# nanoporetech/qcat

Hardware: AMD Instinct MI355X
Metric: reads/sec demultiplexed (higher is better)
Workload: dtype bit planes / int16 (the reference's int32 DP as differences of neighbouring cells in boolean planes: two per difference for the barcode scan, four for the adapter scan of big batches; 16-bit lanes -- u16 / exact-integer f16 -- for the rest; all proven exact per kit by range bounds at kit creation; k

## Files before the change

### include/qcat_hip.h

```cpp
#ifndef QCAT_HIP_H
#define QCAT_HIP_H

#include <stdint.h>

#ifdef __cplusplus
extern "C" {
#endif

#define QCAT_ABI_VERSION 6

enum { QCAT_CODE_A = 0, QCAT_CODE_T = 1, QCAT_CODE_G = 2, QCAT_CODE_C = 3,
       QCAT_CODE_N = 4, QCAT_CODE_X = 5, QCAT_CODE_OTHER = 6, QCAT_CODE_PAD = 7,
       QCAT_NCODES = 7 };

enum { QCAT_MAX_TEMPLATES = 16,
       QCAT_MAX_TEMPLATE_LEN = 128,
       QCAT_MAX_TARGET_LEN = 64,
       QCAT_MAX_BARCODES = 1024,
       QCAT_MAX_WINDOW = 160 };

typedef enum qcat_status {
    QCAT_OK = 0,
    QCAT_ERR_ARG = -1,
    QCAT_ERR_UNSUPPORTED = -2,
// ... 118 lines not shown
                                const int32_t* pair_offsets, const int32_t* pair_entries,
                                const int32_t* quad_offsets, const int32_t* quad_entries);

int  qcat_ctx_create(int device, qcat_ctx** out);
void qcat_ctx_destroy(qcat_ctx* ctx);

int  qcat_scan_batch(qcat_ctx* ctx, const qcat_kit* kit,
                     const uint8_t* bases, const uint64_t* offsets, uint32_t n_reads,
                     qcat_result* out, int64_t* counts);

int  qcat_detect_kit(qcat_ctx* ctx, const qcat_kit* kit,
                     const uint8_t* bases, const uint64_t* offsets, uint32_t n_reads,
                     int64_t* votes, int64_t* first_read);

int  qcat_scan_batch_auto(qcat_ctx* ctx, const qcat_kit* kit,
                          const uint8_t* bases, const uint64_t* offsets, uint32_t n_reads,
                          qcat_result* out, int64_t* counts, int32_t* chosen_kit_slot,
                          int64_t* votes, int64_t* first_read);

int  qcat_scan_batch_auto_ptrs(qcat_ctx* ctx, const qcat_kit* kit,
                               const uint8_t* const* reads, const uint64_t* lengths, uint32_t n_reads,
                               qcat_result* out, int64_t* counts, int32_t* chosen_kit_slot,
                               int64_t* votes, int64_t* first_read);

int  qcat_scan_batches_auto_ptrs(qcat_ctx* ctx, const qcat_kit* kit, const uint8_t* const* reads, const uint64_t* lengths,
                                 uint32_t n_reads, uint32_t batch_reads, qcat_result* out, int64_t* counts,
                                 int32_t* chosen_kit_slots);

int  qcat_scan_sequences(qcat_ctx* ctx, const qcat_kit* kit,
                         const uint8_t* bases, const uint64_t* offsets, uint32_t n_seqs, qcat_result* out);

enum { QCAT_STATS_NONE = 0, QCAT_STATS_PARASAIL6 = 1, QCAT_STATS_PARASAIL5 = 3, QCAT_STATS_ROUND3 = 5 };
typedef struct qcat_alignment { int32_t score, end_query, end_ref, matches, length; } qcat_alignment;
int  qcat_sg_align(qcat_ctx* ctx, const uint8_t* queries, const uint64_t* q_offsets,
                   const uint8_t* targets, const uint64_t* t_offsets, uint32_t n,
                   int32_t gap_open, int32_t gap_extend, const int8_t* matrix , int32_t with_stats,
                   qcat_alignment* out);

int  qcat_scan_debug(qcat_ctx* ctx, const qcat_kit* kit,
                     const uint8_t* bases, const uint64_t* offsets, uint32_t n_reads,
                     qcat_result* out, int64_t* counts,
                     qcat_end_trace* traces, int16_t* bc_rows, uint32_t row_stride);

int  qcat_batch_upload(qcat_ctx* ctx, const uint8_t* bases, const uint64_t* offsets,
                       uint32_t n_reads, qcat_batch** out);
typedef struct qcat_synth_params {
    uint64_t seed;
    uint32_t n_reads;
    uint32_t insert_len;
    uint32_t lead_min, lead_max;
    float    error_rate;
    float    no_adapter_fraction;
    int32_t  tpl_5p, tpl_3p;
} qcat_synth_params;
int  qcat_batch_synthesize(qcat_ctx* ctx, const qcat_kit* kit, const qcat_synth_params* p,
                           qcat_batch** out);
void qcat_batch_destroy(qcat_batch* batch);
int  qcat_batch_info(const qcat_batch* batch, uint32_t* n_reads, uint64_t* n_bases);
int  qcat_batch_download(qcat_ctx* ctx, const qcat_batch* batch, uint8_t* bases, uint64_t* offsets);
int64_t qcat_synth_read(const qcat_kit* kit, const qcat_synth_params* p, uint64_t index,
                        uint8_t* buf, uint64_t cap);

int  qcat_scan_resident(qcat_ctx* ctx, const qcat_kit* kit, const qcat_batch* batch);
int  qcat_ctx_synchronize(qcat_ctx* ctx);
int  qcat_ctx_fetch_results(qcat_ctx* ctx, qcat_result* out, uint32_t n_reads);
int  qcat_ctx_fetch_counts(qcat_ctx* ctx, int64_t* counts, int32_t n_buckets);
void* qcat_ctx_counts_devptr(qcat_ctx* ctx);
void* qcat_ctx_results_devptr(qcat_ctx* ctx);

int  qcat_kit_partition_bins(const qcat_kit* kit);
int  qcat_batch_partition(qcat_ctx* ctx, const qcat_kit* kit, const qcat_batch* batch,
                          const qcat_result* records, uint32_t flags, qcat_batch** out);
int  qcat_ctx_fetch_partition(qcat_ctx* ctx, uint64_t* bin_first, int32_t n_bins, uint32_t* source);
void* qcat_ctx_partition_bins_devptr(qcat_ctx* ctx);
void* qcat_ctx_partition_source_devptr(qcat_ctx* ctx);

void* qcat_ctx_stream(qcat_ctx* ctx);

int64_t qcat_ctx_graph_replays(const qcat_ctx* ctx);

int qcat_ctx_barcode_bitslice_tiles(qcat_ctx* ctx, uint32_t out[3]);
int64_t qcat_ctx_tiny_ends(const qcat_ctx* ctx);
int qcat_ctx_fused_front(const qcat_ctx* ctx, uint32_t out[2]);
int64_t qcat_ctx_middle_wave_reads(qcat_ctx* ctx);

int qcat_ctx_middle_bitslice_tiles(qcat_ctx* ctx, uint32_t out[4]);

int  qcat_ctx_last_timing(qcat_ctx* ctx, const char** names, float* ms, int cap);
int  qcat_ctx_set_timing(qcat_ctx* ctx, int enabled);

int  qcat_set_option(const char* name, int64_t value);
int  qcat_clear_option(const char* name);
int  qcat_get_option(const char* name, int64_t* value);
void qcat_reset_options(void);
int  qcat_option_count(void);
const char* qcat_option_name(int index);
const char* qcat_option_doc(int index);
const char* qcat_backend(void);

typedef struct qcat_fastq qcat_fastq;
int  qcat_fastq_open(const char* path, qcat_fastq** out, uint64_t* n_reads, uint64_t* n_bytes);
void qcat_fastq_close(qcat_fastq* f);
int  qcat_fastq_read_info(const qcat_fastq* f, uint64_t r, uint64_t* title_off, uint32_t* title_len,
                          uint64_t* seq_off, uint32_t* seq_len);
typedef struct qcat_demux_opts {
    int32_t batch_size;
    int32_t kit_auto;
    int32_t trim;
    int32_t min_read_length;
    int32_t tsv;
    int32_t tsv_fd;
    int32_t out_fd;
    const char* out_dir;
    const char* const* kit_name;
    const char* const* const* bc_name;
    const int32_t* const* bc_id;
    const int32_t* const* bc2_id;
    int32_t filter_barcodes;
    int32_t stream_reader;
    uint64_t segment_bytes;
    uint64_t range_begin, range_end;
    int32_t input_fd, rest_fd;
} qcat_demux_opts;
typedef struct qcat_demux_stats {
    uint64_t n_reads, n_skipped, file_bytes;
    double parse_s, scan_s, write_s;
    double total_s;
    uint64_t next_offset;
    int32_t incomplete;
    int32_t segments;
} qcat_demux_stats;
int  qcat_fastq_demux(qcat_fastq* f, qcat_ctx* ctx, const qcat_kit* kit, const qcat_demux_opts* opts,
                      qcat_result* recs, uint8_t* skipped, qcat_demux_stats* stats);

typedef struct qcat_demux_hist {
    int32_t w0, w1;
    int64_t* barcode;
    int64_t* adapter;
    int64_t n_none;
    int64_t n_adapter_none;
} qcat_demux_hist;
int  qcat_fastq_batch_offsets(const char* path, uint32_t batch_size, uint64_t segment_bytes, uint64_t** offsets,
                              uint64_t* n_batches, uint64_t* n_reads, uint64_t* next_offset);
void qcat_free(void* p);
int  qcat_fastq_demux_stream(const char* path, qcat_ctx* ctx, const qcat_kit* kit, const qcat_demux_opts* opts,
                             qcat_demux_hist* hist, qcat_demux_stats* stats);
int  qcat_fastq_stream_count(const char* path, uint64_t segment_bytes, uint32_t batch_size, int32_t stream_reader, uint64_t* n_reads,
                             uint64_t* n_bases, uint64_t* next_offset, uint32_t* n_segments);

enum { QCAT_COMM_ID_BYTES = 128, QCAT_COMM_MAX_VALUES = 64 };
enum { QCAT_REDUCE_SUM = 0, QCAT_REDUCE_MAX = 1 };
typedef struct qcat_comm qcat_comm;
int  qcat_comm_unique_id(uint8_t* id );
int  qcat_comm_create(qcat_ctx* ctx, int n_ranks, int rank, const uint8_t* id, qcat_comm** out);
void qcat_comm_destroy(qcat_comm* comm);
int  qcat_comm_info(const qcat_comm* comm, int* n_ranks, int* rank, int* device);
int  qcat_counts_allreduce(qcat_ctx* ctx, qcat_comm* comm);
int  qcat_comm_allreduce_f64(qcat_ctx* ctx, qcat_comm* comm, double* values, int n, int op);
int  qcat_comm_barrier(qcat_ctx* ctx, qcat_comm* comm);

#ifdef __cplusplus
}
#endif
#endif
```

### qcat_amd/csrc/kernels_abs.inc

```

#include "abs_core.h"
#ifndef QCAT_ABS_NO_BUILTIN
#include "abs_generated.inc"
#endif

namespace qk {

#ifndef QCAT_ABS_TILE_DEFINED
#define QCAT_ABS_TILE_DEFINED
constexpr int ABS_TILE = 2048;
#endif
#ifndef QCAT_ABS_R
#define QCAT_ABS_R 6
#endif
constexpr int ABS_R = QCAT_ABS_R;
constexpr int ABS_MAX_ROWS = 150;
#ifndef QCAT_ABS_PLANE_WAVES
#define QCAT_ABS_PLANE_WAVES 8
#endif
constexpr int ABS_PLANE_WAVES = QCAT_ABS_PLANE_WAVES;

template <int LANE>
__device__ __forceinline__ void abs_writelane(u32 value, u32& acc) {
    asm volatile("v_writelane_b32 %0, %1, %2" : "+v"(acc) : "s"(value), "n"(LANE));
// ... 97 lines not shown
constexpr uint32_t PP_GROUPS = PP_ENDS / 32;
constexpr uint32_t PP_GSTRIDE = 32 * WIN2_WORDS + 4;
static_assert(PP_ITER * PP_THREADS == PP_ENDS * PACK_PARTS && PP_THREADS % PACK_PARTS == 0 && ABS_TILE % PP_ENDS == 0 && PP_ENDS % PK_TILE == 0 &&
              PP_GROUPS * WIN2_WORDS + PP_GROUPS <= PP_THREADS && PACK_CODES == 32, "k_pack_planes: the item arithmetic below");

template <int ENDS>
__global__ void __launch_bounds__(PP_THREADS)
k_pack_planes(const uint8_t* __restrict__ bases, const uint64_t* __restrict__ offsets, uint32_t n_reads, int max_align,
              uint8_t* __restrict__ win, int32_t* __restrict__ wlen, uint8_t* __restrict__ wspec, uint32_t* __restrict__ win2, int lazy_bytes,
              uint2* __restrict__ planes, uint32_t* __restrict__ valid, uint8_t* __restrict__ need128, uint32_t* __restrict__ tile_any) {
    __shared__ __attribute__((aligned(8))) u32 s_win[PP_GROUPS * PP_GSTRIDE];
    __shared__ u32 s_bad[PP_GROUPS];
    const uint64_t n_ends = (uint64_t)n_reads * ENDS;
    const uint64_t e0 = (uint64_t)blockIdx.x * PP_ENDS;
    const uint32_t tile = (uint32_t)(e0 / ABS_TILE), lane0 = (uint32_t)(e0 % ABS_TILE) / 32u;
    if (e0 >= n_ends) {
        if (threadIdx.x < PP_GROUPS) valid[(size_t)tile * 64 + lane0 + threadIdx.x] = 0u;
        return;
    }
    if (threadIdx.x < PP_GROUPS) s_bad[threadIdx.x] = 0u;
    __syncthreads();
    {
        const uint32_t wl = threadIdx.x / PACK_PARTS, part = threadIdx.x - wl * PACK_PARTS;
#pragma unroll
        for (uint32_t it = 0; it < PP_ITER; ++it) {
            const uint32_t el = it * (PP_THREADS / PACK_PARTS) + wl;
            const uint64_t e = e0 + el;
            uint32_t p[PACK_CODES / 16] = {0u, 0u};
            if (e < n_ends && dev_pack_part<ENDS>(bases, offsets, max_align, e, part, win, wlen, wspec, win2, lazy_bytes, p))
                atomicOr(&s_bad[el >> 5], 1u << (el & 31u));
            *reinterpret_cast<uint2*>(&s_win[(el >> 5) * PP_GSTRIDE + (el & 31u) * WIN2_WORDS + part * (PACK_CODES / 16)]) = make_uint2(p[0], p[1]);
        }
    }
    __syncthreads();
    const int rows = max_align;
    if (threadIdx.x < PP_GROUPS * WIN2_WORDS) {
        const uint32_t g = threadIdx.x % PP_GROUPS, d = threadIdx.x / PP_GROUPS;
        u32 v[32];
#pragma unroll
        for (int i = 0; i < 32; ++i) v[i] = s_win[g * PP_GSTRIDE + (uint32_t)i * WIN2_WORDS + d];
        bs_transpose32(v);
        uint2* __restrict__ dst = planes + ((size_t)tile * rows + d * 16u) * 64 + lane0 + g;
#pragma unroll
        for (int q = 0; q < 16; ++q)
            if ((int)(d * 16u) + q < rows) dst[(size_t)q * 64] = make_uint2(v[2 * q + 1], v[2 * q]);
    } else if (threadIdx.x < PP_GROUPS * WIN2_WORDS + PP_GROUPS) {
        const uint32_t g = threadIdx.x - PP_GROUPS * WIN2_WORDS;
        const uint64_t eg = e0 + g * 32u;
        const u32 in = eg >= n_ends ? 0u : (n_ends - eg >= 32u ? 0xFFFFFFFFu : (1u << (uint32_t)(n_ends - eg)) - 1u);
        const u32 ok = in & ~s_bad[g];
        valid[(size_t)tile * 64 + lane0 + g] = ok;
        if (in & ~ok) need128[eg / PK_TILE] = 1;
        if (ok) tile_any[tile] = 1;
    }
}

__device__ __forceinline__ void abs_setprio(int mode, int row, int wg) {
    if (mode == 0) return;
    const int bit = ((row >> (mode - 1)) ^ wg ^ (wg >> 3)) & 1;
    if (bit) __builtin_amdgcn_s_setprio(1); else __builtin_amdgcn_s_setprio(0);
}

template <class P, int S>
constexpr bool abs_is_n(int j) {
    if constexpr (S == 0) return P::N0[j] != 0;
    else if constexpr (S == 1) return P::N1[j] != 0;
    else return P::N[j] != 0;
}
template <class P, int S, int J = 0, int NC>
__device__ __forceinline__ void abs_set2_cols(u32 (&h)[NC][4]) {
    if constexpr (J < NC) {
        if constexpr (abs_is_n<P, S>(J)) qabs::abs_set2_n(h[J]); else qabs::abs_set2(h[J]);
        abs_set2_cols<P, S, J + 1>(h);
    }
}
template <class P, int S, int J = 0, int NC>
__device__ __forceinline__ void abs_hold2_cols(u32 (&h)[NC][4], u32 hold) {
    if constexpr (J < NC) {
        if constexpr (abs_is_n<P, S>(J)) qabs::abs_hold2_n(h[J], hold); else qabs::abs_hold2(h[J], hold);
        abs_hold2_cols<P, S, J + 1>(h, hold);
    }
}

template <class P>
__device__ __forceinline__ void abs_body(const AbsArgs& A) {
    using namespace qabs;
    constexpr int NH = P::NH, NT = P::NT;
    constexpr int PL = 2 + 4 * NH;
    constexpr int LR_WORDS = 2 * ABS_NF + 1;
    static_assert(NH * LR_WORDS <= ABS_R * PL, "the last-row hand-over must fit a ring buffer");
    __shared__ u32 ring[2][ABS_R * PL * 64];
    __shared__ int s_item[2][2];
    const int lane = threadIdx.x & 63, wave = uni((int)(threadIdx.x >> 6));
    const int L = A.rows;
    const int NB = (L + ABS_R - 1) / ABS_R;

    if (wave == 0) {
        u32 h[P::NC0][4];
        int tile = -1, blk = 0;
        constexpr int ABS_PF = 3;
        uint2 pf[ABS_PF];
        const uint2* __restrict__ src = A.planes + lane;
        for (int step = 0;; ++step) {
            const int buf = step & 1;
            if (tile < 0 || blk > NB) {
                for (;;) {
                    u32 t = 0;
                    if (lane == 0) t = atomicAdd(A.cursor, 1u);
                    t = (u32)uni((int)t);
                    if (t >= A.n_tiles) { tile = -1; break; }
                    if (A.tile_any[t]) { tile = (int)t; break; }
                }
                blk = 0;
                if (tile >= 0) {
                    abs_set2_cols<P, 0>(h);
                    src = A.planes + ((size_t)tile * L) * 64 + lane;
#pragma unroll
                    for (int r = 0; r < ABS_PF; ++r) pf[r] = src[(size_t)min(r, L - 1) * 64];
                }
            }
            if (lane == 0) { s_item[buf][0] = tile; s_item[buf][1] = blk; }
            if (tile < 0) { __syncthreads(); __syncthreads(); break; }
            u32* __restrict__ rb = ring[buf];
            if (blk < NB) {
#pragma unroll 1
                for (int r = 0; r < ABS_R; ++r) {
                    const int i = blk * ABS_R + r;
                    if (i < L) {
                        abs_setprio(A.prio, i, (int)blockIdx.x);
                        const uint2 c = pf[0];
#pragma unroll
                        for (int q = 0; q + 1 < ABS_PF; ++q) pf[q] = pf[q + 1];
                        pf[ABS_PF - 1] = src[(size_t)min(i + ABS_PF, L - 1) * 64];
                        u32 nq[4], ho[NH][4];
                        abs_neq_masks(c.x, c.y, nq);
                        P::row0(nq, h, ho);
                        u32* __restrict__ row = rb + r * PL * 64 + lane;
                        row[0] = c.x; row[64] = c.y;
#pragma unroll
                        for (int k = 0; k < NH; ++k)
#pragma unroll
                            for (int p = 0; p < 4; ++p) row[(2 + 4 * k + p) * 64] = ho[k][p];
                    }
                }
            } else {
                AbsLastRow lo[NH];
                P::last0(h, lo);
#pragma unroll
                for (int k = 0; k < NH; ++k) {
                    u32* __restrict__ w = rb + k * LR_WORDS * 64 + lane;
#pragma unroll
                    for (int q = 0; q < ABS_NF; ++q) { w[q * 64] = lo[k].Fr[q]; w[(ABS_NF + q) * 64] = lo[k].sum[q]; }
                    w[2 * ABS_NF * 64] = lo[k].newmax;
                }
            }
            ++blk;
            __syncthreads();
        }
    } else {
        u32 h[P::NC1][4];
        AbsBorder bd[NT];
        __syncthreads();
        for (int step = 1;; ++step) {
            const int buf = (step - 1) & 1;
            const int tile = uni(s_item[buf][0]), blk = uni(s_item[buf][1]);
            if (tile < 0) { __syncthreads(); break; }
            const u32* __restrict__ rb = ring[buf];
            if (blk == 0) {
                abs_set2_cols<P, 1>(h);
#pragma unroll
                for (int t = 0; t < NT; ++t) {
#pragma unroll
                    for (int q = 0; q < ABS_NF; ++q) bd[t].Fc[q] = 0u;
#pragma unroll
                    for (int q = 0; q < ABS_NI; ++q) bd[t].ic[q] = 0u;
                }
            }
            if (blk < NB) {
#pragma unroll 1
                for (int r = 0; r < ABS_R; ++r) {
                    const int i = blk * ABS_R + r;
                    if (i < L) {
                        abs_setprio(A.prio, i + 1, (int)blockIdx.x);
                        const u32* __restrict__ row = rb + r * PL * 64 + lane;
                        u32 nq[4], hi[NH][4];
                        abs_neq_masks(row[0], row[64], nq);
#pragma unroll
                        for (int k = 0; k < NH; ++k)
#pragma unroll
                            for (int p = 0; p < 4; ++p) hi[k][p] = row[(2 + 4 * k + p) * 64];
                        P::row1(nq, h, hi, bd, i == 0 ? 0xFFFFFFFFu : 0u, (unsigned)i);
                    }
                }
            } else {
                AbsLastRow li[NH], lr[NT];
#pragma unroll
                for (int k = 0; k < NH; ++k) {
                    const u32* __restrict__ w = rb + k * LR_WORDS * 64 + lane;
#pragma unroll
                    for (int q = 0; q < ABS_NF; ++q) { li[k].Fr[q] = w[q * 64]; li[k].sum[q] = w[(ABS_NF + q) * 64]; }
                    li[k].newmax = w[2 * ABS_NF * 64];
                }
                P::last1(h, li, lr);
                const u32 keep = A.valid[(size_t)tile * 64 + lane];
#pragma unroll
                for (int t = 0; t < NT; ++t) {
                    u32 val[ABS_NF + 1], endq[ABS_NI];
                    abs_decide(bd[t], lr[t], (unsigned)(L - 1), val, endq, A.r1_scalar != 0);
                    const int M = t == 0 ? P::M0 : P::M1;
                    const int den = A.den[t], tpl = A.tpl[t];
                    AdapterBest* __restrict__ out = A.bests[t] + (size_t)tile * ABS_TILE + (size_t)lane * 32;
                    for (int bit = 0; bit < 32; ++bit) {
                        if (!((keep >> bit) & 1u)) continue;
                        int v = 0, e = 0;
#pragma unroll
                        for (int q = 0; q <= ABS_NF; ++q) v |= (int)((val[q] >> bit) & 1u) << q;
#pragma unroll
                        for (int q = 0; q < ABS_NI; ++q) e |= (int)((endq[q] >> bit) & 1u) << q;
                        const int score = v - 2 * M - 1;
                        if (A.dbg_tpl) {
                            const size_t eidx = (size_t)tile * ABS_TILE + (size_t)lane * 32 + (size_t)bit;
                            A.dbg_tpl[(eidx * 2 + 0) * MAX_T + tpl] = score;
                            A.dbg_tpl[(eidx * 2 + 1) * MAX_T + tpl] = e;
                        }
                        AdapterBest best; best.raw = -1; best.den = 100; best.end = -1; best.tpl = -1;
                        if (best.raw * den < score * best.den) { best.raw = score; best.den = den; best.end = e; best.tpl = tpl; }
                        out[bit] = best;
                    }
                }
            }
            __syncthreads();
        }
    }
}

template <class P>
__global__ void __launch_bounds__(128, 2)
k_adapter_bs(AbsArgs a) { abs_body<P>(a); }

template <class P, class SS, int SI>
__device__ __forceinline__ void abs_stage(const AbsArgs& A, u32* __restrict__ rings, int (*s_item)[2]) {
    using namespace qabs;
    constexpr int NS = P::NS;
    constexpr int LR_WORDS = 2 * ABS_NF + 1;
    static_assert(LR_WORDS <= ABS_R * 4, "a last-row hand-over must fit the ring rows of its difference");
    const int lane = threadIdx.x & 63;
    const int L = A.rows;
    const int NB = (L + ABS_R - 1) / ABS_R;
    constexpr int PLI = 4 * SS::HI, PLO = 4 * SS::HO;
    u32* const ring_in = SS::NHI ? rings + (size_t)SS::RING_IN * ABS_R * 64 : rings;
    u32* const ring_out = SS::NHO ? rings + (size_t)SS::RING_OUT * ABS_R * 64 : rings;
    u32 h[SS::NC][4];
    AbsBorder bd[SS::BD];
    constexpr int ABS_PF = 3;
    uint2 pf[ABS_PF];
    const uint2* __restrict__ src = A.planes + lane;
    int tile = -1, blk = 0;
    for (int step = 0;; ++step) {
        if (step < SI) { __syncthreads(); continue; }
        if (SI == 0) {
            if (tile < 0 || blk > NB) {
                for (;;) {
                    u32 t = 0;
                    if (lane == 0) t = atomicAdd(A.cursor, 1u);
                    t = (u32)uni((int)t);
                    if (t >= A.n_tiles) { tile = -1; break; }
                    if (A.tile_any[t]) { tile = (int)t; break; }
                }
                blk = 0;
            }
            if (lane == 0) { s_item[step & 7][0] = tile; s_item[step & 7][1] = blk; }
        } else {
            tile = uni(s_item[(step - SI) & 7][0]); blk = uni(s_item[(step - SI) & 7][1]);
        }
        if (tile < 0) {
            for (int q = 0; q < NS - 1 - SI; ++q) __syncthreads();
            break;
        }
        if (blk == 0) {
            abs_set2_cols<SS, 2>(h);
#pragma unroll
            for (int t = 0; t < SS::BD; ++t) {
#pragma unroll
                for (int q = 0; q < ABS_NF; ++q) bd[t].Fc[q] = 0u;
#pragma unroll
                for (int q = 0; q < ABS_NI; ++q) bd[t].ic[q] = 0u;
            }
            src = A.planes + ((size_t)tile * L) * 64 + lane;
#pragma unroll
            for (int r = 0; r < ABS_PF; ++r) pf[r] = src[(size_t)min(r, L - 1) * 64];
        }
        const u32* __restrict__ rin = ring_in + (size_t)((step - 1) & 1) * ABS_R * PLI * 64;
        u32* __restrict__ rout = ring_out + (size_t)(step & 1) * ABS_R * PLO * 64;
        if (blk < NB) {
#pragma unroll 1
            for (int r = 0; r < ABS_R; ++r) {
                const int i = blk * ABS_R + r;
                if (i < L) {
                    const uint2 c = pf[0];
#pragma unroll
                    for (int q = 0; q + 1 < ABS_PF; ++q) pf[q] = pf[q + 1];
                    pf[ABS_PF - 1] = src[(size_t)min(i + ABS_PF, L - 1) * 64];
                    u32 nq[4], hi[SS::HI][4], ho[SS::HO][4];
                    if (SS::NHI) {
#pragma unroll
                        for (int k = 0; k < SS::HI; ++k)
#pragma unroll
                            for (int p = 0; p < 4; ++p) hi[k][p] = rin[(r * PLI + 4 * k + p) * 64 + lane];
                    }
                    abs_neq_masks(c.x, c.y, nq);
                    SS::row(nq, h, hi, ho, bd, i == 0 ? 0xFFFFFFFFu : 0u, (unsigned)i);
                    if (SS::NHO) {
#pragma unroll
                        for (int k = 0; k < SS::HO; ++k)
// ... 84 lines not shown
```

### qcat_amd/csrc/kernels_generic.inc

```

namespace qk {

constexpr int GEN_THREADS = 64;
constexpr int GEN_NEG = -(1 << 28);

struct DevAlign { int score, end_q, end_r; };

struct WinSeq {
    const uint8_t* p;
    __device__ __forceinline__ int operator()(int i) const { return p[i]; }
};
struct MidSeq {
    const uint8_t* read; int64_t len; int n; int rev; int off;
    __device__ __forceinline__ int operator()(int i) const {
        const int64_t idx = (int64_t)off + i;
        uint32_t c = rev ? dev_code_of(read[len - n - 1 - idx]) : dev_code_of(read[n + idx]);
        if (rev && c < 4) c ^= 1u;
        return (int)c;
    }
};

template <class Q>
__device__ inline DevAlign dev_sg_generic(const Q q, int L,
                                          const uint8_t* __restrict__ t, int M,
// ... 21 lines not shown
    if (cmax > a.score || (cmax == a.score && (a.end_r == M - 1 || r1_scalar))) {
        a.score = cmax; a.end_r = M - 1; a.end_q = ci - 1;
    }
    return a;
}

__device__ inline uint8_t dev_code_of_ascii(uint8_t c) {
    switch (c & 0xDF) {
        case 'A': return QCAT_CODE_A;
        case 'T': return QCAT_CODE_T;
        case 'G': return QCAT_CODE_G;
        case 'C': return QCAT_CODE_C;
        case 'N': return QCAT_CODE_N;
        case 'X': return QCAT_CODE_X;
        default: return QCAT_CODE_OTHER;
    }
}

struct SgMatrix { int8_t m[49]; };

__global__ void __launch_bounds__(GEN_THREADS)
k_sg_align(const uint8_t* __restrict__ q, const uint64_t* __restrict__ qoff, const uint8_t* __restrict__ t,
           const uint64_t* __restrict__ toff, uint32_t n, int open, int ext, SgMatrix mat, int with_stats_and_rule,
           int32_t* __restrict__ scratch , qcat_alignment* __restrict__ out) {
    const int with_stats = with_stats_and_rule & 0xFF;
    const bool r1_scalar = (with_stats_and_rule & QCAT_SG_R1_SCALAR) != 0;
    const uint32_t a = blockIdx.x * blockDim.x + threadIdx.x;
    const size_t stride = (size_t)gridDim.x * blockDim.x;
    if (a >= n) return;
    const uint8_t* s1 = q + qoff[a];
    const uint8_t* s2 = t + toff[a];
    const int L = (int)(qoff[a + 1] - qoff[a]), M = (int)(toff[a + 1] - toff[a]);
    qcat_alignment r; r.score = 0; r.end_query = -1; r.end_ref = -1; r.matches = 0; r.length = 0;
    if (L <= 0 || M <= 0 || M > MAX_TLEN) { out[a] = r; return; }
    int32_t* H = scratch + a;
    int32_t* F = H + (size_t)(MAX_TLEN + 1) * stride;
    int32_t* HM = F + (size_t)(MAX_TLEN + 1) * stride;
    int32_t* HL = HM + (size_t)(MAX_TLEN + 1) * stride;
    int32_t* FM = HL + (size_t)(MAX_TLEN + 1) * stride;
    int32_t* FL = FM + (size_t)(MAX_TLEN + 1) * stride;
    for (int j = 0; j <= M; ++j) { H[j * stride] = 0; F[j * stride] = GEN_NEG; if (with_stats) { HM[j * stride] = 0; HL[j * stride] = 0; FM[j * stride] = 0; FL[j * stride] = 0; } }
    int cmax = GEN_NEG, cfirst = 0, cm = 0, cl = 0;
    for (int i = 1; i <= L; ++i) {
        const uint8_t c1 = s1[i - 1];
        const int qc = dev_code_of_ascii(c1);
        int diag = 0, dm = 0, dl = 0, hleft = 0, hlm = 0, hll = 0, e = GEN_NEG, em = 0, el = 0;
        for (int j = 1; j <= M; ++j) {
            const uint8_t c2 = s2[j - 1];
            const int tc = dev_code_of_ascii(c2);
            if (hleft - open > e - ext) { e = hleft - open; em = hlm; el = hll + 1; } else { e = e - ext; el = el + 1; }
            const int up = H[j * stride], fo = F[j * stride];
            int f, fm = 0, fl = 0;
            if (up - open > fo - ext) { f = up - open; if (with_stats) { fm = HM[j * stride]; fl = HL[j * stride] + 1; } }
            else { f = fo - ext; if (with_stats) { fm = FM[j * stride]; fl = FL[j * stride] + 1; } }
            int h = diag + mat.m[tc * 7 + qc];
            const int qm = (with_stats == QCAT_STATS_PARASAIL5 && qc == QCAT_CODE_X) ? QCAT_CODE_OTHER : qc;
            const int tm = (with_stats == QCAT_STATS_PARASAIL5 && tc == QCAT_CODE_X) ? QCAT_CODE_OTHER : tc;
            const bool same = with_stats == QCAT_STATS_ROUND3 ? (qc == tc && (c1 | 0x20) == (c2 | 0x20)) : qm == tm;
            int hm = dm + (same ? 1 : 0), hl = dl + 1;
            if (with_stats == QCAT_STATS_ROUND3) {
                if (e > h) { h = e; hm = em; hl = el; }
                if (f > h) { h = f; hm = fm; hl = fl; }
            } else {
                if (f > h) { h = f; hm = fm; hl = fl; }
                if (e > h) { h = e; hm = em; hl = el; }
            }
            diag = up;
            if (with_stats) { dm = HM[j * stride]; dl = HL[j * stride]; HM[j * stride] = hm; HL[j * stride] = hl; FM[j * stride] = fm; FL[j * stride] = fl; }
            H[j * stride] = h; F[j * stride] = f;
            hleft = h; hlm = hm; hll = hl;
        }
        if (hleft > cmax) { cmax = hleft; cfirst = i; cm = hlm; cl = hll; }
    }
    int score = GEN_NEG, end_q = L - 1, end_r = 0, mm = 0, ll = 0;
    for (int j = 1; j <= M; ++j) {
        const int v = H[j * stride];
        if (v > score) { score = v; end_r = j - 1; if (with_stats) { mm = HM[j * stride]; ll = HL[j * stride]; } }
    }
    if (cmax > score || (cmax == score && (end_r == M - 1 || r1_scalar))) { score = cmax; end_r = M - 1; end_q = cfirst - 1; mm = cm; ll = cl; }
    r.score = score; r.end_query = end_q; r.end_ref = end_r; r.matches = with_stats ? mm : 0; r.length = with_stats ? ll : 0;
    out[a] = r;
}

__device__ __host__ inline void dev_region(int tpl_len, int bc_end, int bc_len, int ext, int stop, int L,
                                           int* start_out, int* len_out) {
    int end_ref = stop - (tpl_len - bc_end) + 1;
    int start_ref = end_ref - bc_len;
    start_ref -= (ext < start_ref) ? ext : start_ref;
    end_ref += (ext < L - end_ref) ? ext : (L - end_ref);
    int a = start_ref, b = end_ref + 1;
    if (a < 0) { a += L; if (a < 0) a = 0; }
    if (b < 0) { b += L; if (b < 0) b = 0; }
    if (a > L) a = L;
    if (b > L) b = L;
    *start_out = a;
    *len_out = b > a ? b - a : 0;
}

__global__ void __launch_bounds__(GEN_THREADS)
k_scan_generic(KitPtrs kp, const uint8_t* __restrict__ win, const int32_t* __restrict__ wlen,
               uint32_t n_ends, EndRec* __restrict__ recs,
               int32_t* __restrict__ dbg_tpl ,
               int16_t* __restrict__ dbg_rows , uint32_t stride,
               int adapter_only) {
    __shared__ int H[(MAX_TLEN + 1) * GEN_THREADS];
    __shared__ int F[(MAX_TLEN + 1) * GEN_THREADS];
    __shared__ int8_t amat[49], bmat[49];
    const DevKit* k = kp.kit;
    if (threadIdx.x < 49) { amat[threadIdx.x] = k->amat[threadIdx.x]; bmat[threadIdx.x] = k->bmat[threadIdx.x]; }
    __syncthreads();
    uint32_t e = blockIdx.x * GEN_THREADS + threadIdx.x;
    if (e >= n_ends) return;
    int* h = H + threadIdx.x;
    int* f = F + threadIdx.x;
    const uint8_t* w = win + (size_t)e * WIN_STRIDE;
    const int L = wlen[e];

    int best = -1, best_end = -1, best_raw = -1, best_den = 100;
    if (L > 0) {
        for (int t = 0; t < k->nt; ++t) {
            const DevTpl& p = k->tpl[t];
            DevAlign a = dev_sg_generic(WinSeq{w}, L, kp.codes + p.code_off, p.len, k->gap_open, k->gap_extend, amat, h, f, k->r1_scalar != 0);
            if (dbg_tpl) {
                dbg_tpl[((size_t)e * 2 + 0) * MAX_T + t] = a.score;
                dbg_tpl[((size_t)e * 2 + 1) * MAX_T + t] = a.end_q;
            }
            if ((int64_t)best_raw * p.den < (int64_t)a.score * best_den) {
                best = t; best_end = a.end_q; best_raw = a.score; best_den = p.den;
            }
        }
    }
    EndRec r;
    r.window_len = L; r.best_tpl = best; r.best_end = best_end; r.best_raw = best_raw;
    r.used_tpl = best < 0 ? k->nt - 1 : best;
    const DevTpl& p = k->tpl[r.used_tpl];
    const bool dual = k->mode == QCAT_MODE_DUAL;
    r.region_path = (dual || p.is_double || (best >= 0 && best_raw >= p.region_min_raw)) ? 1 : 0;
    for (int s = 0; s < 2; ++s) { r.region_start[s] = 0; r.region_len[s] = 0; r.bc_idx[s] = -1; r.bc_raw[s] = 0; }
    const int nsets = adapter_only ? 0 : (dual ? 2 : 1);
    for (int s = 0; s < nsets; ++s) {
        if (r.region_path) dev_region(p.len, p.bc_end[s], p.bc_len[s], k->ext, best_end, L, &r.region_start[s], &r.region_len[s]);
        else { r.region_start[s] = 0; r.region_len[s] = L < k->max_align ? L : k->max_align; }
        const DevSet& bs = p.sets[s];
        int bi = -1, braw = 0;
        if (r.region_len[s] > 0) {
            for (int b = 0; b < bs.n; ++b) {
                DevAlign a = dev_sg_generic(WinSeq{w + r.region_start[s]}, r.region_len[s],
                                            kp.codes + bs.tgt_off + (size_t)b * bs.tlen, bs.tlen, 1, 1, bmat, h, f);
                if (dbg_rows) dbg_rows[((size_t)e * 2 + s) * stride + b] = (int16_t)a.score;
                if (bi < 0 || braw == 0 || braw < a.score) { bi = b; braw = a.score; }
            }
        }
        r.bc_idx[s] = bi; r.bc_raw[s] = braw;
    }
    recs[e] = r;
}

template <class MakeQ>
__device__ inline EndRec dev_scan_any(const KitPtrs& kp, MakeQ make_q, int m, int kit_slot,
                                      const int8_t* amat, const int8_t* bmat, int* h, int* f) {
    const DevKit* k = kp.kit;
    const int n = k->max_align;
    int best = -1, best_end = -1, best_raw = -1, best_den = 100, last = -1;
    for (int t = 0; t < k->nt; ++t) {
        const DevTpl& p = k->tpl[t];
        if (kit_slot >= 0 && p.kit_slot != kit_slot) continue;
        last = t;
        if (m <= 0) continue;
        DevAlign a = dev_sg_generic(make_q(0), m, kp.codes + p.code_off, p.len,
                                    k->gap_open, k->gap_extend, amat, h, f, k->r1_scalar != 0);
        if ((int64_t)best_raw * p.den < (int64_t)a.score * best_den) { best = t; best_end = a.end_q; best_raw = a.score; best_den = p.den; }
    }
    EndRec r;
    r.window_len = m; r.best_tpl = best; r.best_end = best_end; r.best_raw = best_raw;
    r.used_tpl = best < 0 ? last : best;
    const DevTpl& p = k->tpl[r.used_tpl];
    const bool dual = k->mode == QCAT_MODE_DUAL;
    r.region_path = (dual || p.is_double || (best >= 0 && best_raw >= p.region_min_raw)) ? 1 : 0;
    const int nsets = dual ? 2 : 1;
    for (int s = 0; s < 2; ++s) { r.region_start[s] = 0; r.region_len[s] = 0; r.bc_idx[s] = -1; r.bc_raw[s] = 0; }
// ... 133 lines not shown
```

### qcat_amd/csrc/kernels_packed.inc

```

#include "cols_generated.inc"

namespace qk {

typedef unsigned short us2 __attribute__((ext_vector_type(2)));
typedef short ss2 __attribute__((ext_vector_type(2)));
typedef uint32_t u32;

__device__ __forceinline__ us2 as_us2(u32 x) { return __builtin_bit_cast(us2, x); }
__device__ __forceinline__ u32 as_u32(us2 x) { return __builtin_bit_cast(u32, x); }
__device__ __forceinline__ us2 pkmax(us2 a, us2 b) { return __builtin_elementwise_max(a, b); }
__device__ __forceinline__ us2 pkmin(us2 a, us2 b) { return __builtin_elementwise_min(a, b); }
__device__ __forceinline__ us2 pkmax_i16(us2 a, us2 b) {
    return __builtin_bit_cast(us2, __builtin_elementwise_max(__builtin_bit_cast(ss2, a), __builtin_bit_cast(ss2, b)));
}
__device__ __forceinline__ us2 pksubsat(us2 a, us2 b) { return __builtin_elementwise_sub_sat(a, b); }
__device__ __forceinline__ us2 addp(us2 a, us2 b) { return as_us2(as_u32(a) + as_u32(b)); }
__device__ __forceinline__ us2 splat(u32 v) { return as_us2(v | (v << 16)); }
__device__ __forceinline__ us2 pack2(u32 lo, u32 hi) { return as_us2(lo | (hi << 16)); }
__device__ __forceinline__ int uni(int v) { return __builtin_amdgcn_readfirstlane(v); }
__device__ __forceinline__ u32 to_vgpr(u32 s) { u32 v; asm volatile("v_mov_b32 %0, %1" : "=v"(v) : "s"(s)); return v; }
__device__ __forceinline__ u32 opaque_v(u32 x) { asm volatile("" : "+v"(x)); return x; }

__device__ __forceinline__ int wave_max(int v) {
#pragma unroll
    for (int off = 32; off > 0; off >>= 1) v = max(v, __shfl_xor(v, off, 64));
    return uni(v);
}

typedef _Float16 h2 __attribute__((ext_vector_type(2)));
__device__ __forceinline__ h2 as_h2(u32 x) { return __builtin_bit_cast(h2, x); }
__device__ __forceinline__ u32 as_u32(h2 x) { return __builtin_bit_cast(u32, x); }
__device__ __forceinline__ h2 hsplat(float v) { const _Float16 x = (_Float16)v; return h2{x, x}; }
__device__ __forceinline__ h2 hmax(h2 a, h2 b) { return __builtin_elementwise_maximum(a, b); }
__device__ __forceinline__ h2 hmin(h2 a, h2 b) { return __builtin_elementwise_minimum(a, b); }
__device__ __forceinline__ h2 hmax3(h2 a, h2 b, h2 c) { return __builtin_elementwise_maximum(__builtin_elementwise_maximum(a, b), c); }
__device__ __forceinline__ u32 make_sel_h(u32 qb) {
    return ((((qb << 12) | qb) & 0x000F000Fu) << 8) | 0x000C000Cu;
}

constexpr int PK_WAVES = 1;
constexpr int PK_TILE = 128;
constexpr int PK_ROWS = 152;
constexpr int JOB_CLASSES = 7;
constexpr int JOB_HOT = 3;
constexpr int JOB_GROUPS = MAX_T * 2;
constexpr int JOB_BINS = JOB_GROUPS * JOB_CLASSES;
static_assert(JOB_BINS <= 256, "a bin index is one byte of a job word (k_adapter_finish)");

__device__ __host__ __forceinline__ int job_class(int L) { return L <= 48 ? 0 : (L <= 64 ? 1 : (L <= 96 ? 2 : 3)); }
__device__ __forceinline__ int job_class_hot_of(int bs_ok, int max_align, int bs_off, int hot_len, int short_min, int flag, int L, int start) {
    if ((flag == 0 || flag == 2) && bs_ok && bs_off >= 0) {
        const bool interior = flag == 2;
        if (L == max_align && (!interior || start == 0)) return JOB_CLASSES - 1;
        if (L == hot_len && !interior) return JOB_CLASSES - 2;
        if (L < hot_len && L >= short_min && !interior) return JOB_CLASSES - 3;
    }
    return job_class(L);
}
__device__ __forceinline__ u32 make_sel(u32 qb) {
    return (((qb << 12) | qb) & 0x000F000Fu) | 0x0C000C00u;
}

#define QK_SEL_KEY_LO 0x0C050400u
#define QK_SEL_KEY_HI 0x0C070600u

struct JobTables {
    uint32_t hist[JOB_BINS];
    uint32_t cursor[JOB_BINS];
    uint32_t group_tile_start[JOB_GROUPS + 1];
    uint32_t unit_cursor[JOB_GROUPS][8][32];
};

enum { TBL_VGPR = 1, TBL_LDS = 2 };

#define QK_POOL(J) (((J) <= PADMAX) ? spv[((J) <= PADMAX) ? (J) - 1 : 0] : special)

template <int W, int TBL>
__device__ __forceinline__ void adapter_align(const u32* __restrict__ tsrc, int M, int g, int Lmax,
                                              const uint8_t* qbuf, int lane, us2 gL2, u32 special,
                                              u32 sel_klo, u32 sel_khi, u32* ltbl, u32 (&rk)[2], u32 (&ck)[2]) {
    const int start = W - M;
    u32 tbl[TBL == TBL_LDS ? 1 : W];
    if constexpr (TBL == TBL_LDS) {
        for (int j = lane; j < W; j += 64) ltbl[j] = tsrc[j];
    } else {
#pragma unroll
        for (int j = 0; j < W; ++j) tbl[j] = tsrc[j];
#pragma unroll
        for (int j = 0; j < W; ++j) tbl[j] = opaque_v(tbl[j]);
    }
    u32 spv[PADMAX];
#pragma unroll
    for (int j = 0; j < PADMAX; ++j) spv[j] = (j + 1 > start) ? special : 0u;
    us2 h[W + 1];
    const us2 g2 = as_us2(opaque_v(as_u32(splat((u32)g))));
    {
        us2 r = splat((u32)(-(g * start)) & 0xFFFFu);
        h[0] = splat(0);
#pragma unroll
        for (int j = 1; j <= W; ++j) { r = r + g2; h[j] = pkmax_i16(r, splat(0)); }
    }
    ck[0] = ck[1] = 0;
    us2 h0old = splat(0);
    u32 qb = qbuf[lane];
    for (int i = 1; i <= Lmax; ++i) {
        if constexpr (TBL == TBL_LDS) asm volatile("" ::: "memory");
        const u32 qb_next = qbuf[(i < PK_ROWS ? i : PK_ROWS - 1) * 64 + lane];
        const u32 sel = make_sel(qb);
        const us2 h0new = pkmin(splat((u32)(g * i)), gL2);
        us2 left = h0new, carry = h0old;
#define QK_W(J) as_us2(__builtin_amdgcn_perm(QK_POOL(J), (TBL == TBL_LDS ? ltbl[(J) - 1] : tbl[TBL == TBL_LDS ? 0 : (J) - 1]), sel))
#define QK_FENCE() if constexpr (TBL == TBL_LDS) asm volatile("" ::: "memory");
#define QK_T us2
#define QK_ADD(a, b) addp(a, b)
#define QK_MAX3(d, u, l) pkmax(pkmax(d, u), l)
        QK_ROW_COLS_DISPATCH(W)
#undef QK_MAX3
#undef QK_ADD
#undef QK_T
#undef QK_FENCE
#undef QK_W
        const u32 dcol = as_u32(left - h0new);
        const u32 ci = (u32)(255 - i);
        ck[0] = max(ck[0], __builtin_amdgcn_perm(dcol, ci, sel_klo));
        ck[1] = max(ck[1], __builtin_amdgcn_perm(dcol, ci, sel_khi));
        h0old = h0new;
        qb = qb_next;
    }
    rk[0] = rk[1] = 0;
    {
        us2 r = splat((u32)(-(g * start) - 1) & 0xFFFFu);
        u32 cj = to_vgpr(255u);
#pragma unroll
        for (int j = 1; j <= W; ++j) {
            r = r + g2;
            cj -= 1u;
            const u32 v = as_u32(pksubsat(h[j], r));
            rk[0] = max(rk[0], __builtin_amdgcn_perm(v, cj, sel_klo));
            rk[1] = max(rk[1], __builtin_amdgcn_perm(v, cj, sel_khi));
        }
    }
}

struct AdapterBest { int32_t raw, den, end, tpl; };

template <int W, int TBL>
__global__ void __launch_bounds__(PK_WAVES * 64, W <= 48 ? 4 : (W <= 64 ? 3 : 2))
k_adapter_packed(KitPtrs kp, const uint8_t* __restrict__ win, const int32_t* __restrict__ wlen,
                 uint32_t n_ends, AdapterBest* __restrict__ bests,
                 int32_t* __restrict__ dbg_tpl, int use_static) {
    __shared__ uint8_t qbuf_all[PK_WAVES][PK_ROWS * 64];
    __shared__ __attribute__((aligned(16))) u32 ltbl_all[PK_WAVES][TBL == TBL_LDS ? W : 4];
    const DevKit* __restrict__ k = kp.kit;
    const int wave = threadIdx.x >> 6, lane = threadIdx.x & 63;
    uint8_t* qbuf = qbuf_all[wave];
    u32* ltbl = ltbl_all[wave];
    const uint32_t base = (blockIdx.x * PK_WAVES + wave) * PK_TILE;
    if (base >= n_ends) return;
    const uint32_t e2[2] = {base + lane, base + 64 + lane};
    const bool valid[2] = {e2[0] < n_ends, e2[1] < n_ends};
    int L2[2] = {valid[0] ? wlen[e2[0]] : 0, valid[1] ? wlen[e2[1]] : 0};

    const uint4 padv = make_uint4(0x07070707u, 0x07070707u, 0x07070707u, 0x07070707u);
    for (int c = 0; c < WIN_STRIDE / 16; ++c) {
        uint4 a = valid[0] ? *reinterpret_cast<const uint4*>(win + (size_t)e2[0] * WIN_STRIDE + c * 16) : padv;
        uint4 b = valid[1] ? *reinterpret_cast<const uint4*>(win + (size_t)e2[1] * WIN_STRIDE + c * 16) : padv;
        const u32 aw[4] = {a.x, a.y, a.z, a.w}, bw[4] = {b.x, b.y, b.z, b.w};
#pragma unroll
        for (int q = 0; q < 16; ++q) {
            const u32 lo = (aw[q >> 2] >> (8 * (q & 3))) & 0xFu;
            const u32 hi = (bw[q >> 2] >> (8 * (q & 3))) & 0xFu;
            if (c * 16 + q < PK_ROWS) qbuf[(c * 16 + q) * 64 + lane] = (uint8_t)(lo | (hi << 4));
        }
    }
    const int Lmax = wave_max(max(L2[0], L2[1]));
    const int g = uni(k->gap_open);
    const int nt = uni(k->nt);
    const us2 gL2 = pack2((u32)(g * L2[0]), (u32)(g * L2[1]));
    const u32 special = to_vgpr(k->special_adapter);
    const u32 sel_klo = to_vgpr(QK_SEL_KEY_LO), sel_khi = to_vgpr(QK_SEL_KEY_HI);

    AdapterBest best[2];
#pragma unroll
    for (int hf = 0; hf < 2; ++hf) {
        best[hf].raw = -1; best[hf].den = 100; best[hf].end = -1; best[hf].tpl = -1;
    }
    for (int t = 0; t < nt; ++t) {
        if (uni(k->tpl[t].width) != W) continue;
        if (use_static && uni(k->tpl[t].static_kernel) >= 0) continue;
        const int M = uni(k->tpl[t].len);
        const int den = uni(k->tpl[t].den);
        const u32* __restrict__ tsrc = kp.tables + uni(k->tpl[t].tbl_off);
        u32 rk[2], ck[2];
        adapter_align<W, TBL>(tsrc, M, g, Lmax, qbuf, lane, gL2, special, sel_klo, sel_khi, ltbl, rk, ck);
        const bool r1_scalar = uni(k->r1_scalar) != 0;
        const int start = W - M;
#pragma unroll
        for (int hf = 0; hf < 2; ++hf) {
            const int L = L2[hf];
            if (L > 0) {
                const int vr = (int)(rk[hf] >> 8) - 1, jr = 255 - (int)(rk[hf] & 255u) - start;
                const int vc = (int)(ck[hf] >> 8), ic = 255 - (int)(ck[hf] & 255u);
                const int s_row = vr - g * L, s_col = vc - g * M;
                const bool col = s_col > s_row || (s_col == s_row && (jr == M || r1_scalar));
                const int score = col ? s_col : s_row;
                const int endq = col ? ic - 1 : L - 1;
                if (dbg_tpl) {
                    dbg_tpl[((size_t)e2[hf] * 2 + 0) * MAX_T + t] = score;
                    dbg_tpl[((size_t)e2[hf] * 2 + 1) * MAX_T + t] = endq;
                }
                const int lhs = best[hf].raw * den, rhs = score * best[hf].den;
                if (lhs < rhs || (lhs == rhs && best[hf].tpl >= 0 && t < best[hf].tpl)) {
                    best[hf].raw = score; best[hf].den = den; best[hf].end = endq; best[hf].tpl = t;
                }
            }
        }
    }
#pragma unroll
    for (int hf = 0; hf < 2; ++hf) if (valid[hf]) bests[e2[hf]] = best[hf];
}

__global__ void __launch_bounds__(256)
k_adapter_finish(const DevKit* __restrict__ k, const int32_t* __restrict__ wlen, uint32_t n_ends,
                 const AdapterBest* __restrict__ bests, int n_slices, EndRec* __restrict__ recs,
                 JobTables* __restrict__ jt, const int32_t* __restrict__ fallback_tpl, int kit_mask,
                 const uint8_t* __restrict__ wspec, uint32_t* __restrict__ jobinfo, int2* __restrict__ bcres,
                 uint32_t* __restrict__ fin, const int32_t* __restrict__ kit_slot_dev = nullptr, uint32_t slot_span = 0) {
    if (kit_slot_dev && !slot_span) kit_mask = *kit_slot_dev;
    __shared__ uint32_t hist[JOB_BINS];
    struct FinTpl { int32_t kit_slot, is_double, region_min_raw, len, bc_end[2], bc_len[2], hot_len[2], short_min[2], bs_off[2]; };
    __shared__ FinTpl s_tpl[MAX_T];
    if (threadIdx.x < JOB_BINS) hist[threadIdx.x] = 0;
    const int nt = k->nt;
    if ((int)threadIdx.x < nt) {
        const DevTpl& p = k->tpl[threadIdx.x];
        FinTpl f;
        f.kit_slot = p.kit_slot; f.is_double = p.is_double; f.region_min_raw = p.region_min_raw; f.len = p.len;
#pragma unroll
        for (int s = 0; s < 2; ++s) {
            f.bc_end[s] = p.bc_end[s]; f.bc_len[s] = p.bc_len[s];
            f.hot_len[s] = p.sets[s].hot_len; f.short_min[s] = p.sets[s].bs_short_min; f.bs_off[s] = p.sets[s].bs_off;
        }
        s_tpl[threadIdx.x] = f;
    }
    __syncthreads();
    const bool dual = k->mode == QCAT_MODE_DUAL;
    const int nsets = dual ? 2 : 1;
    const int bs_ok = k->bs_ok, max_align = k->max_align, ext = k->ext;
    for (uint32_t e = blockIdx.x * blockDim.x + threadIdx.x; e < n_ends; e += gridDim.x * blockDim.x) {
        AdapterBest cs[MAX_T];
#pragma unroll
        for (int sl = 0; sl < MAX_T; ++sl) if (sl < n_slices) cs[sl] = bests[(size_t)sl * n_ends + e];
        const int L = wlen[e];
        const int flag = wspec ? (int)wspec[e] : 1;
        const int fb = fallback_tpl ? fallback_tpl[e] : 0;
        if (slot_span) kit_mask = kit_slot_dev[e / slot_span];
        AdapterBest b = cs[0];
        if (kit_mask >= 0 && b.tpl >= 0 && s_tpl[b.tpl].kit_slot != kit_mask) { b.raw = -1; b.den = 100; b.end = -1; b.tpl = -1; }
#pragma unroll
        for (int sl = 1; sl < MAX_T; ++sl) {
            if (sl >= n_slices) break;
            const AdapterBest c = cs[sl];
            if (c.tpl < 0) continue;
            if (kit_mask >= 0 && s_tpl[c.tpl].kit_slot != kit_mask) continue;
            const int lhs = b.raw * c.den, rhs = c.raw * b.den;
            if (lhs < rhs || (lhs == rhs && b.tpl >= 0 && c.tpl < b.tpl)) b = c;
        }
        EndRec r;
        r.window_len = L; r.best_tpl = b.tpl; r.best_end = b.end; r.best_raw = b.raw;
        int last = nt - 1;
        if (kit_mask >= 0) while (last > 0 && s_tpl[last].kit_slot != kit_mask) --last;
        r.used_tpl = b.tpl < 0 ? (fallback_tpl ? fb : last) : b.tpl;
        const FinTpl& p = s_tpl[r.used_tpl];
        r.region_path = (dual || p.is_double || (b.tpl >= 0 && b.raw >= p.region_min_raw)) ? 1 : 0;
        for (int s = 0; s < 2; ++s) { r.region_start[s] = 0; r.region_len[s] = 0; r.bc_idx[s] = -1; r.bc_raw[s] = 0; }
        for (int s = 0; s < nsets; ++s) {
            if (r.region_path) dev_region(p.len, p.bc_end[s], p.bc_len[s], ext, b.end, L, &r.region_start[s], &r.region_len[s]);
            else { r.region_start[s] = 0; r.region_len[s] = L < max_align ? L : max_align; }
            uint32_t ji = 0;
            if (r.region_len[s] > 0 && !(fallback_tpl != nullptr && r.region_len[s] > max_align)) {
                const int bin = (r.used_tpl * 2 + s) * JOB_CLASSES +
                                job_class_hot_of(bs_ok, max_align, p.bs_off[s], p.hot_len[s], p.short_min[s], flag, r.region_len[s], r.region_start[s]);
                atomicAdd(&hist[bin], 1u);
                ji = (uint32_t)min(r.region_len[s], 255) | ((uint32_t)bin << 8) | ((uint32_t)r.region_start[s] << 16);
            }
            jobinfo[(size_t)e * nsets + s] = ji;
            if (bcres) bcres[(size_t)e * nsets + s] = make_int2(-1, 0);
        }
        if (fin) fin[e] = (uint32_t)(r.window_len & 0xFF) | ((uint32_t)(r.used_tpl & 0xFF) << 8) | ((uint32_t)(uint16_t)(int16_t)r.best_end << 16);
        else recs[e] = r;
    }
    __syncthreads();
    if (threadIdx.x < JOB_BINS && hist[threadIdx.x]) atomicAdd(&jt->hist[threadIdx.x], hist[threadIdx.x]);
}

__global__ void k_job_offsets(JobTables* jt) {
    __shared__ uint32_t s_hist[JOB_BINS], s_cur[JOB_BINS], s_grp[JOB_GROUPS + 1];
    if (blockIdx.x != 0) return;
    for (int b = (int)threadIdx.x; b < JOB_BINS; b += (int)blockDim.x) s_hist[b] = jt->hist[b];
    __syncthreads();
    if (threadIdx.x == 0) {
        uint32_t pos = 0;
        for (int gidx = 0; gidx < JOB_GROUPS; ++gidx) {
            const uint32_t gstart = pos;
            s_grp[gidx] = gstart / PK_TILE;
            for (int c = 0; c < JOB_CLASSES; ++c) {
                s_cur[gidx * JOB_CLASSES + c] = pos;
                pos += s_hist[gidx * JOB_CLASSES + c];
            }
            pos = gstart + (pos - gstart + PK_TILE - 1) / PK_TILE * PK_TILE;
        }
        s_grp[JOB_GROUPS] = pos / PK_TILE;
    }
    __syncthreads();
    for (int b = (int)threadIdx.x; b < JOB_BINS; b += (int)blockDim.x) jt->cursor[b] = s_cur[b];
    for (int g = (int)threadIdx.x; g <= JOB_GROUPS; g += (int)blockDim.x) jt->group_tile_start[g] = s_grp[g];
}

constexpr int SCAT_PER_THREAD = 8;
__global__ void __launch_bounds__(256)
k_job_scatter(const uint32_t* __restrict__ jobinfo, uint32_t n_ends, int nsets,
              JobTables* __restrict__ jt, int32_t* __restrict__ sorted, uint32_t* __restrict__ posof) {
    __shared__ uint32_t cnt[JOB_BINS], basep[JOB_BINS];
    if (threadIdx.x < JOB_BINS) cnt[threadIdx.x] = 0;
    __syncthreads();
    const uint32_t n_cand = n_ends * (uint32_t)nsets;
    const uint32_t blk0 = blockIdx.x * 256u * SCAT_PER_THREAD;
    int key[SCAT_PER_THREAD]; uint32_t rank[SCAT_PER_THREAD];
#pragma unroll
    for (int it = 0; it < SCAT_PER_THREAD; ++it) {
        const uint32_t id = blk0 + it * 256u + threadIdx.x;
        key[it] = -1; rank[it] = 0;
        if (id < n_cand) {
            const uint32_t ji = jobinfo[id];
            if (ji) {
                key[it] = (int)((ji >> 8) & 0xFFu);
                rank[it] = atomicAdd(&cnt[key[it]], 1u);
            }
        }
    }
    __syncthreads();
    if (threadIdx.x < JOB_BINS && cnt[threadIdx.x]) basep[threadIdx.x] = atomicAdd(&jt->cursor[threadIdx.x], cnt[threadIdx.x]);
    __syncthreads();
#pragma unroll
    for (int it = 0; it < SCAT_PER_THREAD; ++it)
    {
        const uint32_t id = blk0 + it * 256u + threadIdx.x;
        if (key[it] >= 0) {
            const uint32_t pos = basep[key[it]] + rank[it];
            sorted[pos] = (int32_t)id;
            if (posof) posof[id] = pos;
        } else if (posof && id < n_cand) posof[id] = 0xFFFFFFFFu;
    }
}

struct TileMeta { uint32_t e_lo, e_hi, len2, pad; };
struct BsPlan;
__device__ __forceinline__ bool bs_covers(const BsPlan* __restrict__ bp, int gidx, uint32_t tile);
__device__ __forceinline__ void bs_uncovered_runs(const BsPlan* __restrict__ bp, uint32_t t0, uint32_t t1, int gidx, uint32_t (&start)[4], uint32_t (&len)[4]);

constexpr int GATHER_THREADS = 64 * (WIN_STRIDE / 16);
__global__ void __launch_bounds__(GATHER_THREADS)
k_job_gather(const uint8_t* __restrict__ win, const uint32_t* __restrict__ jobinfo, const int32_t* __restrict__ sorted,
             const JobTables* __restrict__ jt, int nsets, uint8_t* __restrict__ tilebuf, TileMeta* __restrict__ tmeta,
             const BsPlan* __restrict__ taken ,
             const uint32_t* __restrict__ win2 = nullptr, const uint8_t* __restrict__ wspec = nullptr ) {
    const uint32_t chunks = WIN_STRIDE / 16;
    const uint32_t chunk = threadIdx.x % chunks, lane = threadIdx.x / chunks;
    const uint32_t n_tiles = jt->group_tile_start[JOB_GROUPS];
    auto image = [&](uint32_t tile) {
        const int32_t id2[2] = {sorted[(size_t)tile * PK_TILE + lane], sorted[(size_t)tile * PK_TILE + 64 + lane]};
        uint32_t e2[2] = {0, 0};
        int L2[2] = {0, 0}, st2[2] = {0, 0};
#pragma unroll
        for (int hf = 0; hf < 2; ++hf) {
            if (id2[hf] >= 0) {
// ... 385 lines not shown
        __syncthreads();
        if (threadIdx.x == 0) {
            int bi = -1, braw = 0;
            for (int b = 0; b < bs.n; ++b) {
                const int raw = score[b];
                if (bi < 0 || braw == 0 || braw < raw) { bi = b; braw = raw; }
            }
            if (bcres) bcres[(size_t)e * (k->mode == QCAT_MODE_DUAL ? 2 : 1) + set] = make_int2(bi, braw);
            else { recs[e].bc_idx[set] = bi; recs[e].bc_raw[set] = braw; }
        }
        __syncthreads();
    }
}

constexpr int QCAT_JIT_BASE = 1 << 20;
enum { QCAT_JIT_ADAPTER = 0, QCAT_JIT_MIDDLE = 1, QCAT_JIT_BARCODE = 2, QCAT_JIT_BITSLICE = 3,
       QCAT_JIT_ABS2 = 4, QCAT_JIT_ABSM = 5, QCAT_JIT_ABSW = 6 };
#ifndef QCAT_RTC
static inline void jit_launch(int kind, int index, dim3 grid, hipStream_t stream, const void* args);
#endif

struct StaticArgs {
    KitPtrs kp;
    const uint8_t* tilebuf;
    const TileMeta* tmeta;
    JobTables* jt;
    u32* raws;
    int bstride, chunk_b, gidx, xcd_queues;
    u32* part;
    int part_stride;
    const BsPlan* bs;
};
struct StaticBarcodeMulti {
    StaticArgs common;
    int16_t gidx[JOB_GROUPS], chunk_b[JOB_GROUPS];
    int16_t kernel[JOB_GROUPS];
    int32_t n;
};
#ifndef QCAT_RTC
static inline void launch_barcode_static(int kernel, dim3 grid, hipStream_t stream, const StaticArgs& a);
static inline void launch_barcode_multi(dim3 grid, hipStream_t stream, const StaticBarcodeMulti& m);
#endif
struct StaticAdapterArgs {
    KitPtrs kp;
    const uint8_t* win;
    const int32_t* wlen;
    uint32_t n_ends;
    AdapterBest* bests;
    int32_t* dbg_tpl;
    int tpl;
    AdapterBest* bests2;
    int tpl2;
    const uint8_t* only;
    const uint32_t* win2;
    const uint8_t* wspec;
};

struct FillList { int32_t n; uint32_t word[8]; void* p[8]; unsigned long long bytes[8]; };
__global__ void __launch_bounds__(256)
k_fill_multi(FillList f) {
    for (int r = 0; r < f.n; ++r) {
        const unsigned long long n16 = f.bytes[r] / 16;
        const uint4 v = make_uint4(f.word[r], f.word[r], f.word[r], f.word[r]);
        uint4* __restrict__ q = reinterpret_cast<uint4*>(f.p[r]);
        for (unsigned long long i = (unsigned long long)blockIdx.x * blockDim.x + threadIdx.x; i < n16; i += (unsigned long long)gridDim.x * blockDim.x) q[i] = v;
        const unsigned tail = (unsigned)(f.bytes[r] - n16 * 16);
        if (blockIdx.x == 0 && threadIdx.x < tail) reinterpret_cast<uint8_t*>(f.p[r])[n16 * 16 + threadIdx.x] = (uint8_t)f.word[r];
    }
}

struct AbsArgs {
    const uint2* planes;
    const uint32_t* valid;
    const uint32_t* tile_any;
    AdapterBest* bests[2];
    int32_t tpl[2];
    int32_t den[2];
    uint32_t n_ends, n_tiles;
    int32_t rows;
    uint32_t* cursor;
    int32_t* dbg_tpl;
    int32_t prio;
    int32_t r1_scalar;
};
struct StaticAdapterMulti {
    StaticAdapterArgs common;
    AdapterBest* bests[MAX_T];
    AdapterBest* bests2[MAX_T];
    int16_t tpl[MAX_T], tpl2[MAX_T];
    int16_t kernel[MAX_T];
    int16_t fused[MAX_T];
};
#ifndef QCAT_RTC
static inline void launch_adapter_static(int kernel, dim3 grid, hipStream_t stream, const StaticAdapterArgs& a);
static inline void launch_adapter_fused(int kernel, dim3 grid, hipStream_t stream, const StaticAdapterArgs& a);
static inline void launch_adapter_multi(dim3 grid, hipStream_t stream, const StaticAdapterMulti& m);
#endif

}
```

### qcat_amd/csrc/options.h

```cpp
#ifndef QCAT_OPTIONS_H
#define QCAT_OPTIONS_H
#ifndef QCAT_RTC
#include <atomic>
#include <stdint.h>
#include <stdlib.h>

#define QCAT_OPTION_LIST(X) \
    X(NO_STATIC, "1: no generated static-letter kernels (binary16 table kernels instead)") \
    X(NO_STATIC_ADAPTER, "1: the adapter templates on the table kernels") \
    X(NO_FUSED_ADAPTER, "1: the two templates of a kit as two launches instead of the fused kernel") \
    X(NO_BARCODE_MULTI, "1: the static-letter barcode kernels of a small batch as launches of their own instead of one (k_barcode_multi)") \
    X(NO_ADAPTER_MULTI, "1: the static-letter adapter kernels of a small batch as launches of their own instead of one (k_adapter_multi)") \
    X(BARCODE_U16, "1 at kit creation: u16 lanes instead of exact-integer binary16 for the barcode tables") \
    X(NO_BITSLICE, "1: every barcode alignment on the binary16 kernels") \
    X(NO_BS_STATIC, "1: bit-sliced barcode kernels with the letters from memory") \
    X(BITSLICE_MIN, "barcode alignments from which the bit-sliced path is taken (default: 40 000 + 1 900 000 / barcodes; dual kits 70 000 + 3 500 000 / barcodes)") \
    X(BITSLICE_PAD, "jobs from which the rest of a hot class becomes a padded super-tile (0 / unset: never)") \
    X(BS_NO_SOLO, "1: no producer waves for the shared columns") \
    X(BS_NO_SHORT, "1: regions a few bases short of nominal stay on the binary16 kernels (no front-padded units)") \
    X(BS_SIDE, "1: ... on side streams whatever the batch size") \
    X(LEFTOVER_SIDE, "0 / 1: the left-over binary16 tiles behind / beside the bit-sliced launches") \
    X(BS_DRAW, "0 / 1: the waves of a bit-sliced workgroup take a unit's barcodes round robin / draw them from a counter (default 1; sets of 32 barcodes or more)") \
    X(BS_TRACE, "1: print the phase boundaries of one workgroup and the unit log of the bit-sliced launches") \
    X(BS_TRACE_UNITS, "1: ... and every unit") \
    X(BS_TRACE_WG, "the workgroup whose phase boundaries BS_TRACE prints (default 0)") \
    X(BS_TRACE_SEQ, "... from its n-th unit on (eight units; default 0)") \
    X(CHUNK_BARCODES, "barcodes per work unit of the binary16 barcode kernels") \
    X(ONE_QUEUE, "1: one unit queue instead of XCD-local ones") \
    X(ONE_STREAM, "1: no side streams") \
    X(RAWS, "1: keep the per-barcode raw score array (no summary keys)") \
    X(SUMMARY, "1: summary keys for small barcode sets as well") \
    X(NO_ADAPTER_BITSLICE, "1: the adapter scan on the binary16 kernels") \
    X(ADAPTER_BITSLICE_MIN, "read ends from which the bit-sliced adapter scan is taken") \
    X(ABS_STAGES, "2 / 4: one form of the adapter plans for every batch size") \
    X(FORCE_GENERIC, "1 at context creation: the general int32 kernel for everything") \
    X(MIDDLE_GENERIC, "1: --detect-middle on the general kernel") \
    X(MIDDLE_NO_ABS, "1: the interior adapter scan on the binary16 kernel") \
    X(MIDDLE_ABS_MIN, "slots from which the bit-sliced interior adapter scan is taken") \
    X(MIDDLE_ABS_ROWS, "rows of the interior's plane buffer") \
    X(MIDDLE_ABS_ONE_WAVE, "0 / 1: two-wave pipeline / one wave per big tile") \
    X(NO_PIPELINE, "1: no chunked host pipeline") \
    X(PIPELINE_CHUNK, "reads per chunk of the host pipeline") \
    X(PIPELINE_TRACE, "1: print the split of a pipelined call") \
    X(NO_SIMPLE_PACKED, "1: simple mode on the general kernel (k_scan_simple) instead of the packed end-tracking kernels") \
    X(NO_TINY, "1: batches of a handful of read ends take the throughput kernels like every other batch") \
    X(TINY_MAX_ENDS, "largest batch (read ends, at most 4096) on the one-wave-per-alignment kernels (default: by the number of alignments, 20000)") \
    X(WAVE_MAX, "most alignments of a call (pairs of qcat_sg_align without statistics; sequences of qcat_scan_sequences with affine gap costs, sequences x barcodes with a simple list) that take the one-wave kernels (default: the limits in kernels_tiny.inc)") \
    X(AUTO_CHUNK, "batches per call of the kit-auto file loop") \
    X(AUTO_WORKERS, "contexts of the kit-auto file loop") \
    X(NO_GRAPH, "1: host-buffer calls never replay a captured graph") \
    X(DEBUG_VOTE, "1: print the kit vote") \
    X(DEBUG_BINS, "1: print the jobs per length class") \
    X(DEBUG_REDO, "1: print how many alignments took the sequential arg-max")

#define QCAT_AB_OPTION_LIST(X) \
    X(NO_QUADS, "1 at kit creation: static barcode chains as pairs only") \
    X(BS_STATIC_MIN, "super-tiles from which the generated bit-sliced kernels are taken") \
    X(BS_FROM_TILES, "1: bit-sliced units read tile images instead of the two-bit windows") \
    X(BS_NO_TAIL_SPLIT, "1: the last round of long units is not cut into barcode chunks") \
    X(BS_SERIAL, "1: the bit-sliced launches of a scan in line on the context's stream") \
    X(NO_SLIM, "1: the 60-byte per-end records instead of the packed result arrays") \
    X(NO_FILL_MERGE, "1: one fill launch per buffer instead of k_fill_multi") \
    X(EAGER_BYTES, "1: byte windows for every read end, not only for those with a letter outside A, C, G, T") \
    X(PACK_PLANES, "0: windows and adapter letter planes of a big batch as two kernels (k_pack_windows, k_abs_planes) instead of one (k_pack_planes)") \
    X(FIN_BLOCKS, "blocks of k_finalize") \
    X(FINISH_BLOCKS, "blocks of k_adapter_finish") \
    X(ABS_NO_SPLIT, "1: medium batches keep the fused two-template plan") \
    X(ABS_PRIO, "issue priority rotation of the bit-sliced adapter kernels") \
    X(ADAPTER_REVERSE, "1: the side-by-side adapter launches in reverse order") \
    X(MIDDLE_NO_BITSLICE, "1: the interior's barcode jobs on the binary16 kernels") \
    X(MIDDLE_ABS_WINDOWS, "0: the M-ends' first windows from the reads instead of the packed batch") \
    X(MIDDLE_ABS_WGS, "workgroups per CU of the interior adapter kernels") \
    X(MIDDLE_ABS_EARLY, "1: the packed batch at the start of the scan") \
    X(MIDDLE_ABS_PRIO, "issue priority rotation of the interior adapter kernels") \
    X(FULL_UPLOAD, "1: host-buffer calls upload whole reads") \
    X(ABS_SERIAL, "1: the bit-sliced adapter launches of a scan one after the other instead of side by side (A/B)") \
    X(NO_ZERO_COPY, "1: host-buffer calls of a handful of reads copy their staging to the device like bigger ones (A/B)") \
    X(STREAM_SYNC_RELEASE, "1: the file loop's reader gives a written segment's pages back itself (A/B: a thread of its own)")

enum QcatOpt {
#define X(N, D) QO_##N,
    QCAT_OPTION_LIST(X)
    QO_PUBLIC_COUNT,
    QO_AB_BASE_ = QO_PUBLIC_COUNT - 1,
    QCAT_AB_OPTION_LIST(X)
#undef X
    QO_COUNT
};
#ifdef QCAT_AB
constexpr int QO_SETTABLE = QO_COUNT;
#else
constexpr int QO_SETTABLE = QO_PUBLIC_COUNT;
#endif

constexpr int64_t QOPT_UNSET = INT64_MIN;
extern std::atomic<int64_t> g_qcat_opt[QO_COUNT];

struct QOptVal {
    bool set;
    int64_t v;
    explicit operator bool() const { return set; }
};
inline QOptVal qopt_get(QcatOpt o) { if ((int)o >= QO_SETTABLE) return QOptVal{false, 0}; const int64_t v = g_qcat_opt[o].load(std::memory_order_relaxed); return QOptVal{v != QOPT_UNSET, v == QOPT_UNSET ? 0 : v}; }
inline bool opt_is_set(QcatOpt o) { return (int)o < QO_SETTABLE && g_qcat_opt[o].load(std::memory_order_relaxed) != QOPT_UNSET; }
inline bool opt_on(QcatOpt o) { if ((int)o >= QO_SETTABLE) return false; const int64_t v = g_qcat_opt[o].load(std::memory_order_relaxed); return v != QOPT_UNSET && v != 0; }
inline int64_t opt_val(QcatOpt o, int64_t dflt) { if ((int)o >= QO_SETTABLE) return dflt; const int64_t v = g_qcat_opt[o].load(std::memory_order_relaxed); return v == QOPT_UNSET ? dflt : v; }
inline int atoi(const QOptVal& o) { return (int)o.v; }
inline long long atoll(const QOptVal& o) { return (long long)o.v; }
#endif
#endif
```

### qcat_amd/csrc/packed_host.inc

```

#include "dev_buf.h"

extern "C" void qcat_abs_launch_planes(unsigned n_tiles, void* stream, const uint32_t* win2, const int32_t* wlen, const uint8_t* wspec,
                                       uint32_t n_ends, int rows, void* planes, uint32_t* valid, uint8_t* need128, uint32_t* tile_any);
extern "C" unsigned qcat_abs_launch_pack_planes(void* stream, const uint8_t* bases, const uint64_t* offsets, uint32_t n_reads, int ends, int rows,
                                                uint8_t* win, int32_t* wlen, uint8_t* wspec, uint32_t* win2, int lazy_bytes,
                                                void* planes, uint32_t* valid, uint8_t* need128, uint32_t* tile_any);
extern "C" int qcat_abs_launch(int kind, int id, unsigned grid, void* stream, const void* args);

namespace qk {

#ifndef QCAT_ABS_TILE_DEFINED
#define QCAT_ABS_TILE_DEFINED
constexpr int ABS_TILE = 2048;
#endif
constexpr int RESUME_KIT_ON_DEVICE = 1 << 20;

struct PackedScratch {
    DevBuf<JobTables> jt;
    DevBuf<int32_t> sorted;
    DevBuf<uint32_t> jobinfo;
    DevBuf<AdapterBest> bests;
    int n_slices = 0;
    bool slices_single = false;
    DevBuf<uint8_t> tilebuf;
    DevBuf<TileMeta> tmeta;
    DevBuf<uint32_t> raws;
    DevBuf<uint32_t> part;
    DevBuf<uint32_t> redo;
    const uint8_t* wspec = nullptr;
    const uint8_t* win = nullptr;
    const uint32_t* win2 = nullptr;
    bool lazy = false;
    DevBuf<BsPlan> bsplan;
    DevBuf<uint32_t> bskeys;
    bool bs_last = false;
    DevBuf<uint2> bsrp;
    DevBuf<uint2> abs_planes;
    DevBuf<uint32_t> abs_valid;
    DevBuf<uint8_t> abs_flags;
    DevBuf<uint32_t> posof;
    DevBuf<int2> bcres;
    bool slim = false;
    DevBuf<uint32_t> fin;
    bool fin_only = false;
    uint32_t abs_ready = 0;
    uint32_t abs_zeroed = 0;
    const int32_t* kit_slot_dev = nullptr;
    uint32_t kit_slot_span = 0;
    bool prepared = false;
    bool redo_zeroed = false;
    static constexpr int NAUX = 11;
    hipStream_t aux[NAUX] = {};
    hipEvent_t ev_fork = nullptr, ev_join[NAUX] = {};
};

static thread_local std::string g_packed_err;
static thread_local FillList g_fill = {};
static thread_local bool g_fill_defer = false;
static inline hipError_t packed_fill(void* p, int byte, size_t bytes, hipStream_t stream) {
    if (g_fill_defer && g_fill.n < 8 && bytes > 0) {
        const uint32_t b = (uint32_t)(byte & 0xFF);
        g_fill.p[g_fill.n] = p; g_fill.bytes[g_fill.n] = bytes; g_fill.word[g_fill.n] = b * 0x01010101u; ++g_fill.n;
        return hipSuccess;
    }
    return bytes ? hipMemsetAsync(p, byte, bytes, stream) : hipSuccess;
}
static inline hipError_t packed_fill_flush(hipStream_t stream) {
    g_fill_defer = false;
    if (g_fill.n == 0) return hipSuccess;
    unsigned long long most = 0;
    for (int r = 0; r < g_fill.n; ++r) most = std::max(most, g_fill.bytes[r]);
    const unsigned blocks = (unsigned)std::min<unsigned long long>(1024, std::max<unsigned long long>(1, most / (16 * 256 * 4)));
    hipLaunchKernelGGL(k_fill_multi, dim3(blocks), dim3(256), 0, stream, g_fill);
    g_fill.n = 0;
    return hipGetLastError();
}
struct FillScope {
    explicit FillScope(bool defer) { g_fill.n = 0; g_fill_defer = defer; }
    ~FillScope() { g_fill.n = 0; g_fill_defer = false; }
    FillScope(const FillScope&) = delete;
    FillScope& operator=(const FillScope&) = delete;
};
static inline const char* packed_last_error() { return g_packed_err.c_str(); }
static thread_local int g_jit_rc = 0;
static inline int jit_take_error() { const int rc = g_jit_rc; g_jit_rc = 0; return rc; }

static inline hipError_t packed_streams(PackedScratch* s) {
    if (s->ev_fork) return hipSuccess;
    hipError_t e = hipEventCreateWithFlags(&s->ev_fork, hipEventDisableTiming);
    for (int i = 0; i < PackedScratch::NAUX && e == hipSuccess; ++i) {
        e = hipStreamCreateWithFlags(&s->aux[i], hipStreamNonBlocking);
        if (e == hipSuccess) e = hipEventCreateWithFlags(&s->ev_join[i], hipEventDisableTiming);
    }
    return e;
}

template <class Launch>
static inline void fork_join(PackedScratch* s, hipStream_t stream, int n, Launch launch) {
    if (n <= 0) return;
    const bool multi = n > 1 && s->ev_fork && !opt_on(QO_ONE_STREAM);
    if (multi) (void)hipEventRecord(s->ev_fork, stream);
    bool used[PackedScratch::NAUX] = {};
    for (int i = 0; i < n; ++i) {
        hipStream_t q = stream;
        if (multi && i > 0) {
            const int a = (i - 1) % PackedScratch::NAUX;
            q = s->aux[a];
            if (!used[a]) { (void)hipStreamWaitEvent(q, s->ev_fork, 0); used[a] = true; }
        }
        launch(i, q);
    }
    for (int a = 0; a < PackedScratch::NAUX; ++a)
        if (used[a]) { (void)hipEventRecord(s->ev_join[a], s->aux[a]); (void)hipStreamWaitEvent(stream, s->ev_join[a], 0); }
}

static inline void packed_streams_reset(PackedScratch* s) {
    for (int i = 0; i < PackedScratch::NAUX; ++i) {
        if (s->aux[i]) (void)hipStreamDestroy(s->aux[i]);
        if (s->ev_join[i]) (void)hipEventDestroy(s->ev_join[i]);
        s->aux[i] = nullptr; s->ev_join[i] = nullptr;
    }
    if (s->ev_fork) (void)hipEventDestroy(s->ev_fork);
    s->ev_fork = nullptr;
}

static inline void packed_scratch_free(PackedScratch* s) { packed_streams_reset(s); }

static inline int packed_max_width(const DevKit& k) {
    int m = 0;
    for (int t = 0; t < k.nt; ++t) m = std::max(m, k.tpl[t].width);
    return m;
// ... 13 lines not shown
    return (int)QCAT_ERR_DEVICE;
}
template <class T>
static inline int packed_ensure(DevBuf<T>& b, size_t n, const char* what) {
    const hipError_t e = b.ensure(n);
    return e == hipSuccess ? 0 : packed_fail(("hipMalloc(" + std::string(what) + ")").c_str(), e);
}

static inline int abs_cu_count() {
    int cus = 256, dev = 0;
    (void)hipGetDevice(&dev);
    (void)hipDeviceGetAttribute(&cus, hipDeviceAttributeMultiprocessorCount, dev);
    return cus;
}
static inline int abs_forms(const DevKit& hk, int t) {
    const int sk = hk.tpl[t].static_kernel;
    if (sk < 0) return 0;
    if (sk >= QCAT_JIT_BASE) return hk.tpl[t].abs_jit;
    return (qcat_abs_launch(1, sk, 0, nullptr, nullptr) ? 1 : 0) | (qcat_abs_launch(2, sk, 0, nullptr, nullptr) ? 2 : 0) |
           (qcat_abs_launch(3, sk, 0, nullptr, nullptr) ? 4 : 0);
}
static inline void abs_launch_form(const DevKit& hk, int t, int form, unsigned grid, hipStream_t q, const AbsArgs& aa) {
    const int sk = hk.tpl[t].static_kernel;
    if (sk >= QCAT_JIT_BASE) jit_launch(form == 1 ? QCAT_JIT_ABS2 : (form == 2 ? QCAT_JIT_ABSM : QCAT_JIT_ABSW), t, dim3(grid), q, &aa);
    else (void)qcat_abs_launch(form == 1 ? 1 : (form == 2 ? 2 : 3), sk, grid, q, &aa);
}
static inline bool packed_abs_wanted(const DevKit& hk, uint32_t n_ends, bool have_wspec) {
    const bool use_static_a = hk.adapter_f16 && !opt_on(QO_NO_STATIC) && !opt_on(QO_NO_STATIC_ADAPTER);
    const QOptVal amin = qopt_get(QO_ADAPTER_BITSLICE_MIN);
    const size_t abs_min = amin ? (size_t)atoll(amin) : (size_t)abs_cu_count() * 7 * ABS_TILE / 2;
    if (!(hk.abs_ok && have_wspec && use_static_a && !opt_on(QO_NO_ADAPTER_BITSLICE))) return false;
    const size_t abs_min_ms = (size_t)abs_cu_count() * 3 * ABS_TILE / 2;
    const bool medium = n_ends < std::max<size_t>(abs_min, 1);
    if (medium && (amin || n_ends < abs_min_ms)) return false;
    bool any = false;
    for (int t = 0; t < hk.nt; ++t) {
        const int forms = abs_forms(hk, t);
        if (medium) { if (!(forms & 2)) return false; any = true; continue; }
        if (forms & 5) any = true;
        if (hk.tpl[t].static_kernel >= 0 && hk.tpl[t].static_kernel < QCAT_JIT_BASE && hk.tpl[t].fused_kernel >= 0 &&
            qcat_abs_launch(0, hk.tpl[t].fused_kernel, 0, nullptr, nullptr) != 0) any = true;
    }
    return any;
}
static inline int packed_abs_buffers(hipStream_t stream, const DevKit& hk, uint32_t n_ends, PackedScratch* sc) {
    hipError_t e;
    int rc;
    const uint32_t abs_tiles = (n_ends + ABS_TILE - 1) / ABS_TILE;
    const size_t need_planes = (size_t)abs_tiles * hk.max_align * 64, need_valid = (size_t)abs_tiles * 64;
    const size_t need_flags = (size_t)MAX_T * 4 + (size_t)abs_tiles * 4 + (size_t)abs_tiles * (ABS_TILE / PK_TILE);
    if ((rc = packed_ensure(sc->abs_planes, need_planes, "adapter letter planes"))) return rc;
    if ((rc = packed_ensure(sc->abs_valid, need_valid, "adapter keep masks"))) return rc;
    if ((rc = packed_ensure(sc->abs_flags, need_flags, "adapter tile flags"))) return rc;
    if ((e = packed_fill(sc->abs_flags, 0, need_flags, stream)) != hipSuccess) return packed_fail("memset(adapter tile flags)", e);
    sc->abs_zeroed = n_ends;
    return 0;
}

static inline int packed_prepare(hipStream_t stream, const DevKit& hk, uint32_t n_ends, PackedScratch* sc) {
    auto fail = packed_fail;
    const int nsets = hk.mode == QCAT_MODE_DUAL ? 2 : 1;
    const size_t n_cand = (size_t)n_ends * nsets;
    const size_t need_sorted = n_cand + (size_t)JOB_GROUPS * PK_TILE;
    hipError_t e;
    int rc;
    if ((rc = packed_ensure(sc->jt, 1, "job tables"))) return rc;
    if ((e = packed_streams(sc)) != hipSuccess) return fail("side streams", e);
    if ((rc = packed_ensure(sc->sorted, need_sorted, "sorted jobs"))) return rc;
    if ((rc = packed_ensure(sc->jobinfo, n_cand, "job words"))) return rc;
    if (sc->slim) {
        if ((rc = packed_ensure(sc->posof, n_cand, "job positions"))) return rc;
        if ((rc = packed_ensure(sc->bcres, n_cand, "barcode results"))) return rc;
        if ((rc = packed_ensure(sc->fin, n_ends, "finalize words"))) return rc;
    }
    if ((e = packed_fill(sc->jt, 0, sizeof(JobTables), stream)) != hipSuccess) return fail("memset(job tables)", e);
    if ((e = packed_fill(sc->sorted, 0xFF, need_sorted * 4, stream)) != hipSuccess) return fail("memset(sorted)", e);
    if (sc->redo && (e = packed_fill(sc->redo, 0, 4, stream)) != hipSuccess) return fail("memset(redo count)", e);
    sc->redo_zeroed = sc->redo != nullptr;

    return 0;
}

static inline int packed_adapter_finish(hipStream_t stream, KitPtrs kp, const uint8_t* , const int32_t* wlen,
                                        uint32_t n_ends, EndRec* recs, PackedScratch* sc, int kit_mask) {
    const QOptVal fb_env = qopt_get(QO_FINISH_BLOCKS);
    const uint32_t fblocks = std::min<uint32_t>((n_ends + 255) / 256, fb_env ? (uint32_t)std::max(1, atoi(fb_env)) : 1024u);
    const int32_t* slot_dev = kit_mask == RESUME_KIT_ON_DEVICE ? sc->kit_slot_dev : nullptr;
    hipLaunchKernelGGL(k_adapter_finish, dim3(fblocks), dim3(256), 0, stream, kp.kit, wlen, n_ends, sc->bests, sc->n_slices, recs, sc->jt,
                       (const int32_t*)nullptr, slot_dev ? -1 : kit_mask, sc->wspec, sc->jobinfo, sc->slim ? sc->bcres : nullptr, sc->fin_only ? sc->fin : nullptr,
                       slot_dev, slot_dev ? sc->kit_slot_span : 0u);
    hipError_t e = hipGetLastError();
    if (e != hipSuccess) return packed_fail("packed kernel launch", e);
    return 0;
}

template <class Mark>
static inline int packed_adapter(hipStream_t stream, KitPtrs kp, const DevKit& hk, const uint8_t* win,
                                 const int32_t* wlen, uint32_t n_ends, EndRec* recs, PackedScratch* sc,
                                 int32_t* dbg_tpl, Mark mark) {
    auto fail = packed_fail;
    hipError_t e;
    int rc;
    const int adapter_widths[] = {40, 48, 56, 60, 64, 84, 92, 104, 112, 120, 128};
    const bool use_static_a = hk.adapter_f16 && !opt_on(QO_NO_STATIC) && !opt_on(QO_NO_STATIC_ADAPTER);
    auto table_tpl = [&](int t, int w) { return hk.tpl[t].width == w && !(use_static_a && hk.tpl[t].static_kernel >= 0); };
    int n_slices = 0, n_static_a = 0;
    for (int w : adapter_widths) { bool present = false; for (int t = 0; t < hk.nt; ++t) present |= table_tpl(t, w); n_slices += present; }
    for (int t = 0; t < hk.nt; ++t) if (use_static_a && hk.tpl[t].static_kernel >= 0) { ++n_slices; ++n_static_a; }
    if ((rc = packed_ensure(sc->bests, (size_t)n_ends * n_slices, "adapter bests"))) return rc;
    const uint32_t tiles = (n_ends + PK_TILE - 1) / PK_TILE;
    const uint32_t blocks = (tiles + PK_WAVES - 1) / PK_WAVES;
    {
        int slice = 0;
#define QK_LAUNCH(WW, TT) do { bool present = false; for (int t = 0; t < hk.nt; ++t) present |= table_tpl(t, WW); \
        if (present) { hipLaunchKernelGGL((k_adapter_packed<WW, TT>), dim3(blocks), dim3(PK_WAVES * 64), 0, stream, kp, win, wlen, n_ends, \
                                          sc->bests + (size_t)slice * n_ends, dbg_tpl, use_static_a ? 1 : 0); ++slice; } } while (0)
        QK_LAUNCH(40, TBL_VGPR); QK_LAUNCH(48, TBL_VGPR); QK_LAUNCH(56, TBL_VGPR); QK_LAUNCH(60, TBL_VGPR); QK_LAUNCH(64, TBL_VGPR);
        QK_LAUNCH(84, TBL_LDS); QK_LAUNCH(92, TBL_LDS); QK_LAUNCH(104, TBL_LDS); QK_LAUNCH(112, TBL_LDS); QK_LAUNCH(120, TBL_LDS); QK_LAUNCH(128, TBL_LDS);
#undef QK_LAUNCH
        if (slice) mark("k_adapter_packed");
        const bool use_fused = !opt_on(QO_NO_FUSED_ADAPTER);
        const uint32_t abs_tiles = (n_ends + ABS_TILE - 1) / ABS_TILE;
        const int abs_cus = abs_cu_count();
        const bool abs_wanted = packed_abs_wanted(hk, n_ends, sc->wspec != nullptr && (sc->win2 != nullptr || sc->abs_ready == n_ends));
        const bool abs_split = abs_wanted && abs_tiles < (uint32_t)abs_cus * 4u && !opt_on(QO_ABS_NO_SPLIT);
        int stpl[MAX_T], sslice[MAX_T], spartner[MAX_T], pslice[MAX_T];
        int ns = 0, nsl = 0;
        bool taken[MAX_T] = {};
        for (int t = 0; t < hk.nt; ++t) {
            if (!(use_static_a && hk.tpl[t].static_kernel >= 0) || taken[t]) continue;
            stpl[ns] = t; sslice[ns] = slice + nsl++; spartner[ns] = -1; pslice[ns] = 0;
            const int p = hk.tpl[t].fused_partner;
            const bool split_pair = abs_split && p > t && hk.tpl[t].static_kernel < QCAT_JIT_BASE &&
                                    (abs_forms(hk, t) & 1) && (abs_forms(hk, p) & 1);
            if (!split_pair && use_fused && hk.tpl[t].fused_kernel >= 0 && hk.tpl[t].static_kernel < QCAT_JIT_BASE && p > t && !taken[p]) {
                spartner[ns] = p; pslice[ns] = slice + nsl++; taken[p] = true;
            }
            ++ns;
        }
        bool abs_plan[MAX_T] = {};
        bool use_abs = false;
        {
            if (abs_wanted)
                for (int i = 0; i < ns; ++i) {
                    const int t = stpl[i];
                    abs_plan[i] = spartner[i] >= 0 ? qcat_abs_launch(0, hk.tpl[t].fused_kernel, 0, nullptr, nullptr) != 0
                                                   : (abs_forms(hk, t) & 5) != 0;
                    use_abs = use_abs || abs_plan[i];
                }
        }
        uint32_t* abs_cursor = nullptr; uint32_t* abs_tile_any = nullptr; uint8_t* abs_need128 = nullptr;
        if (use_abs) {
            const bool ready = sc->abs_ready == n_ends;
            if (!ready && sc->abs_zeroed != n_ends) { const int rc2 = packed_abs_buffers(stream, hk, n_ends, sc); if (rc2) return rc2; }
            sc->abs_zeroed = 0;
            abs_cursor = reinterpret_cast<uint32_t*>(sc->abs_flags.get());
            abs_tile_any = abs_cursor + MAX_T;
            abs_need128 = reinterpret_cast<uint8_t*>(abs_tile_any + abs_tiles);
            if (!ready)
                qcat_abs_launch_planes(abs_tiles, stream, sc->win2, wlen, sc->wspec, n_ends, hk.max_align, sc->abs_planes, sc->abs_valid,
                                       abs_need128, abs_tile_any);
        }
        sc->abs_ready = 0;
        const int abs_prio = (int)opt_val(QO_ABS_PRIO, 0);
        const QOptVal stages_env = qopt_get(QO_ABS_STAGES);
        const bool abs_ms = stages_env ? atoi(stages_env) == 4 : abs_tiles < (uint32_t)abs_cus * 7u / 2u;
        const bool adapter_reverse = opt_on(QO_ADAPTER_REVERSE);
        const bool adapter_serial = opt_on(QO_ABS_SERIAL) && use_abs;
        auto adapter_unit = [&](int i0, hipStream_t q) {
            const int i = adapter_reverse ? ns - 1 - i0 : i0;
            const int t = stpl[i];
            StaticAdapterArgs sa{kp, win, wlen, n_ends, sc->bests + (size_t)sslice[i] * n_ends, dbg_tpl, t,
                                 spartner[i] >= 0 ? sc->bests + (size_t)pslice[i] * n_ends : nullptr, spartner[i],
                                 abs_plan[i] ? abs_need128 : nullptr, sc->lazy ? sc->win2 : nullptr, sc->wspec};
            if (abs_plan[i]) {
                AbsArgs aa{sc->abs_planes, sc->abs_valid, abs_tile_any, {sa.bests, sa.bests2}, {t, spartner[i]},
                           {hk.tpl[t].den, spartner[i] >= 0 ? hk.tpl[spartner[i]].den : 0}, n_ends, abs_tiles, hk.max_align, abs_cursor + i, dbg_tpl, abs_prio, hk.r1_scalar};
                const unsigned grid = (unsigned)std::min<uint32_t>(abs_tiles, (uint32_t)abs_cus * 4u);
                if (spartner[i] >= 0) (void)qcat_abs_launch(0, hk.tpl[t].fused_kernel, grid, q, &aa);
                else {
                    const int forms = abs_forms(hk, t);
                    if (abs_ms && (forms & 2)) abs_launch_form(hk, t, 2, grid, q, aa);
                    else if (forms & 1) abs_launch_form(hk, t, 1, grid, q, aa);
                    else abs_launch_form(hk, t, 4, (unsigned)std::min<uint32_t>(abs_tiles, (uint32_t)abs_cus * 2u), q, aa);
                }
            }
            if (spartner[i] >= 0) launch_adapter_fused(hk.tpl[t].fused_kernel, dim3(tiles), q, sa);
            else launch_adapter_static(hk.tpl[t].static_kernel, dim3(tiles), q, sa);
        };
        bool multi = ns >= 2 && !use_abs && !opt_on(QO_NO_ADAPTER_MULTI) && (uint64_t)tiles * (uint64_t)ns <= (uint64_t)abs_cus * 16u;
        for (int i = 0; i < ns && multi; ++i) multi = hk.tpl[stpl[i]].static_kernel < QCAT_JIT_BASE;
        if (multi) {
            StaticAdapterMulti mm{};
            mm.common = StaticAdapterArgs{kp, win, wlen, n_ends, nullptr, dbg_tpl, 0, nullptr, -1, nullptr, sc->lazy ? sc->win2 : nullptr, sc->wspec};
            for (int i = 0; i < ns; ++i) {
                const int t = stpl[i];
                mm.bests[i] = sc->bests + (size_t)sslice[i] * n_ends;
                mm.bests2[i] = spartner[i] >= 0 ? sc->bests + (size_t)pslice[i] * n_ends : nullptr;
                mm.tpl[i] = (int16_t)t; mm.tpl2[i] = (int16_t)spartner[i];
                mm.fused[i] = spartner[i] >= 0 ? 1 : 0;
                mm.kernel[i] = (int16_t)(spartner[i] >= 0 ? hk.tpl[t].fused_kernel : hk.tpl[t].static_kernel);
            }
            launch_adapter_multi(dim3(tiles, (uint32_t)ns), stream, mm);
        } else if (adapter_serial) for (int i0 = 0; i0 < ns; ++i0) adapter_unit(i0, stream);
        else fork_join(sc, stream, ns, adapter_unit);
        slice += nsl;
        if (n_static_a) mark(use_abs ? "k_adapter_bitslice" : "k_adapter_static");
    }
    sc->n_slices = n_slices;
    sc->slices_single = n_static_a == n_slices;
    if ((e = hipGetLastError()) != hipSuccess) return fail("packed kernel launch", e);
    rc = jit_take_error();
    if (rc) return rc;
    return packed_adapter_finish(stream, kp, win, wlen, n_ends, recs, sc, -1);
}

template <class Mark, class Gather>
static inline int packed_barcode(hipStream_t stream, KitPtrs kp, const DevKit& hk, uint32_t n_ends, EndRec* recs,
                                 PackedScratch* sc, Gather gather, int16_t* dbg_rows, uint32_t stride, Mark mark) {
    auto fail = packed_fail;
    hipError_t e;
    int rc;
    const int nsets = hk.mode == QCAT_MODE_DUAL ? 2 : 1;
    const size_t n_cand = (size_t)n_ends * nsets;
    const size_t need_sorted = n_cand + (size_t)JOB_GROUPS * PK_TILE;
    hipLaunchKernelGGL(k_job_offsets, dim3(1), dim3(128), 0, stream, sc->jt);
    {
        const uint32_t per_block = 256u * SCAT_PER_THREAD;
        const uint32_t sblocks = (uint32_t)((n_cand + per_block - 1) / per_block);
        hipLaunchKernelGGL(k_job_scatter, dim3(sblocks), dim3(256), 0, stream, sc->jobinfo, n_ends, nsets, sc->jt, sc->sorted, sc->slim ? sc->posof : nullptr);
    }
    const uint32_t max_tiles = (uint32_t)(need_sorted / PK_TILE);
    if ((rc = packed_ensure(sc->tilebuf, (size_t)max_tiles * 64 * WIN_STRIDE, "tile images"))) return rc;
    if ((rc = packed_ensure(sc->tmeta, (size_t)max_tiles * 64, "tile meta"))) return rc;
    bool gathered = false;
    auto ensure_gather = [&](const BsPlan* taken) {
        if (gathered) return;
        gather(max_tiles, taken, stream);
        mark("k_job_sort");
        gathered = true;
    };
    {
        int bstride = 1;
        for (int t = 0; t < hk.nt; ++t) for (int s = 0; s < nsets; ++s) bstride = std::max(bstride, (int)hk.tpl[t].sets[s].n);
        const bool use_static0 = hk.barcode_f16 && !opt_on(QO_NO_STATIC);
        bool bs_sets = false;
        for (int t = 0; t < hk.nt; ++t) for (int s = 0; s < nsets; ++s) bs_sets = bs_sets || hk.tpl[t].sets[s].bs_off >= 0;
        const QOptVal bs_min_env = qopt_get(QO_BITSLICE_MIN);
        const size_t bs_min = bs_min_env ? (size_t)atoll(bs_min_env)
                                         : (nsets == 2 ? (size_t)70000 + (size_t)3500000 / (size_t)std::max(1, bstride)
                                                       : (size_t)40000 + (size_t)1900000 / (size_t)std::max(1, bstride));
        const bool bs_direct = !opt_on(QO_BS_FROM_TILES) && sc->win != nullptr && sc->win2 != nullptr;
        const QOptVal pad_env = qopt_get(QO_BITSLICE_PAD);
        int bs_cus = 256;
        { int dev = 0; (void)hipGetDevice(&dev); (void)hipDeviceGetAttribute(&bs_cus, hipDeviceAttributeMultiprocessorCount, dev); }
        const uint32_t bs_pad_min = !bs_direct ? 0u : (pad_env ? (uint32_t)std::max(0, atoi(pad_env)) / PK_TILE * PK_TILE
                                                               : (n_cand / BS_JOBS >= (size_t)bs_cus ? (uint32_t)PK_TILE : 0u));
        const bool small_big_set = pad_env && bs_pad_min > 0 && bstride >= 48 && n_cand >= 2048 && n_cand < std::max<size_t>(bs_min, BS_JOBS) && !bs_min_env;
        const bool bs_wanted = hk.bs_ok && bs_sets && sc->wspec && !opt_on(QO_NO_BITSLICE) &&
                               (n_cand >= std::max<size_t>(bs_min, BS_JOBS) || (small_big_set && bs_pad_min > 0));
        bool summary = use_static0 && dbg_rows == nullptr && !opt_on(QO_RAWS) &&
                       (bstride > 32 || bs_wanted || opt_on(QO_SUMMARY));
        for (int t = 0; t < hk.nt && summary; ++t)
            for (int s = 0; s < nsets; ++s) if (hk.tpl[t].sets[s].static_kernel < 0) { summary = false; break; }
        const size_t need_raws = summary ? 0 : (size_t)max_tiles * bstride * 64;
        if (need_raws && (rc = packed_ensure(sc->raws, need_raws, "raw barcode scores"))) return rc;
        const QOptVal chunk_env = qopt_get(QO_CHUNK_BARCODES);
        const int chunk_b = chunk_env ? std::max(1, atoi(chunk_env)) : 4;
        const int nch = std::max(1, (bstride + chunk_b - 1) / chunk_b);
        const uint32_t bblocks = (uint32_t)(((uint64_t)max_tiles * nch + PK_WAVES - 1) / PK_WAVES);
        const int order = 1;
        const bool use_static = hk.barcode_f16 && !opt_on(QO_NO_STATIC);
        bool have[7] = {false, false, false, false, false, false, false};
        bool any_table = false, any_static = false;
        for (int t = 0; t < hk.nt; ++t)
            for (int s = 0; s < nsets; ++s) {
                if (use_static && hk.tpl[t].sets[s].static_kernel >= 0) { any_static = true; continue; }
                const int w = hk.tpl[t].sets[s].width;
                have[w == 40 ? 0 : (w == 44 ? 1 : (w == 48 ? 2 : (w == 56 ? 3 : (w == 64 ? 4 : (w == 42 ? 5 : 6)))))] = true;
                any_table = true;
            }
        if (any_table) ensure_gather(nullptr);
#define QK_LAUNCH_B(IDX, WW) if (have[IDX]) { \
            if (hk.barcode_f16) hipLaunchKernelGGL((k_barcode_packed<WW, true>), dim3(bblocks), dim3(PK_WAVES * 64), 0, stream, \
                                                   kp, sc->tilebuf, sc->tmeta, sc->jt, sc->raws, bstride, nch, order, use_static ? 1 : 0); \
            else hipLaunchKernelGGL((k_barcode_packed<WW, false>), dim3(bblocks), dim3(PK_WAVES * 64), 0, stream, \
                                    kp, sc->tilebuf, sc->tmeta, sc->jt, sc->raws, bstride, nch, order, use_static ? 1 : 0); }
        QK_LAUNCH_B(0, 40) QK_LAUNCH_B(5, 42) QK_LAUNCH_B(1, 44) QK_LAUNCH_B(6, 46) QK_LAUNCH_B(2, 48) QK_LAUNCH_B(3, 56) QK_LAUNCH_B(4, 64)
#undef QK_LAUNCH_B
        if (any_table) mark("k_barcode_packed");
        if (any_static) {
            int dev = 0, cus = 256;
            (void)hipGetDevice(&dev);
            (void)hipDeviceGetAttribute(&cus, hipDeviceAttributeMultiprocessorCount, dev);
            const uint32_t persist = (uint32_t)cus * 16u;
            int sgrp[JOB_GROUPS];
            int ng = 0;
// ... 203 lines not shown
```

### qcat_amd/csrc/qcat_hip.hip

```cpp
#include <hip/hip_runtime.h>

#include <sched.h>

#include <algorithm>
#include <atomic>
#include <memory>
#include <cctype>
#include <chrono>
#include <cstdio>
#include <cstring>
#include <map>
#include <mutex>
#include <string>
#include <thread>
#include <vector>

#include "kit.h"
#include "synth.h"

#include "kit_prepare.inc"
#include "kernels_common.inc"
#include "kernels_generic.inc"
#include "kernels_tiny.inc"
#include "kernels_packed.inc"
// ... 641 lines not shown
    sc->wspec = mid_bs ? c->mid_wspec : nullptr;
    sc->win2 = mid_bs ? c->mid_win2 : nullptr;
    sc->win = c->win;
    sc->lazy = mid_bs;
    sc->slim = false;
    FillScope fills(merge_fills);
    if ((rc = packed_prepare(st, hk, (uint32_t)slots, sc))) return set_err(rc, packed_last_error());
    const uint32_t tiles = (uint32_t)(slots / PK_TILE);
    AbsMidArgs am{};
    bool use_absm = false;
    c->absm_last_big = 0; c->absm_last_128 = 0;
    {
        const uint32_t kmask = absmid_wanted(hk, n);
        if (kmask) {
            const uint32_t big = (uint32_t)((slots + 2047) / 2048);
            const QOptVal rcap = qopt_get(QO_MIDDLE_ABS_ROWS);
            size_t rows = rcap ? (size_t)atoll(rcap)
                               : std::min<size_t>((size_t)1 << 30, (size_t)(2 * b->n_bases / 2048) * 5 / 4 + (size_t)big * 128 + 16384 + 64);
            if (!rcap && rows * 64 > c->absm_planes.cap()) {
                size_t free_b = 0, total_b = 0;
                if (hipMemGetInfo(&free_b, &total_b) == hipSuccess) rows = std::min(rows, std::max<size_t>(16384, free_b / 4 / 768));
            }
            const size_t tw = (size_t)big * (4 + 128) + MAX_T;
            if ((rc = grow(c->absm_tiles, tw))) return rc;
            if ((rc = grow(c->absm_need, (size_t)tiles + 16))) return rc;
            if ((rc = grow(c->absm_planes, rows * 64))) return rc;
            if ((rc = grow(c->absm_ns, rows * 64))) return rc;
            constexpr size_t C2_SLACK = ABSM_C2_SLACK_HOST;
            const bool early = c->absm_codes_early;
            c->absm_codes_early = false;
            if (!early) {
                if ((rc = grow(c->absm_c2, (size_t)(b->n_bases / 16) + 4 + 2 * C2_SLACK))) return rc;
                if ((rc = grow(c->absm_rspec, (size_t)n + 1))) return rc;
            }
            if ((rc = grow(c->absm_sinfo, slots))) return rc;
            uint32_t* w = c->absm_tiles;
            am.bases = b->bases; am.offsets = b->offsets; am.msorted = c->mid_sorted; am.mlen = c->mid_len; am.mt = c->mid_tables;
            am.max_align = hk.max_align; am.n_tiles = big; am.slot_cap = (uint32_t)slots; am.nt = hk.nt; am.kit_mask = kmask;
            am.t_rows = (int32_t*)w; am.t_pz = (int32_t*)(w + big); am.t_kit = (int32_t*)(w + 2 * (size_t)big); am.t_off = w + 3 * (size_t)big;
            am.nonempty = w + 4 * (size_t)big; am.invalid = w + 4 * (size_t)big + 64 * (size_t)big;
            am.cursor = w + (size_t)big * (4 + 128);
            am.c2 = c->absm_c2 + C2_SLACK; am.rspec = c->absm_rspec; am.sinfo = c->absm_sinfo; am.n_bases = b->n_bases; am.n_reads = n;
            if (early) HIPCHK(hipStreamWaitEvent(st, c->absm_done, 0));
            else HIPCHK(packed_fill(c->absm_rspec, 0, (size_t)n + 1, st));
            am.need128 = c->absm_need; am.planes = c->absm_planes; am.ns = c->absm_ns; am.row_cap = (uint32_t)rows;
            am.bests = c->mid_bests; am.tpl = -1; am.den = 0; am.kit_slot = -1;
            const QOptVal pr = opt_is_set(QO_MIDDLE_ABS_PRIO) ? qopt_get(QO_MIDDLE_ABS_PRIO) : qopt_get(QO_ABS_PRIO);
            am.prio = pr ? atoi(pr) : 2;
            am.r1_scalar = hk.r1_scalar;
            HIPCHK(packed_fill(am.cursor, 0, MAX_T * 4, st));
            HIPCHK(packed_fill_flush(st));
            const bool c2win = mid_bs && !((opt_is_set(QO_MIDDLE_ABS_WINDOWS) && opt_val(QO_MIDDLE_ABS_WINDOWS, 0) == 0));
            fork_join(sc, st, (mid_bs && !c2win) ? 2 : 1, [&](int i, hipStream_t q) {
                if (i == 0) qcat_absmid_prepare(q, &am, c2win ? c->mid_win2 : nullptr, c2win ? c->mid_wspec : nullptr, early ? 2 : 3); else launch_mid_windows(q);
            });
            use_absm = true;
            c->absm_last_big = big; c->absm_last_128 = tiles;
        }
    }
    HIPCHK(packed_fill_flush(st));
    int absm_side = 0;
    if (use_absm) for (int t = 0; t < hk.nt; ++t) if ((am.kit_mask >> hk.tpl[t].kit_slot) & 1u) ++absm_side;
    if (mid_bs && !use_absm) launch_mid_windows(st);
    fork_join(sc, st, hk.nt, [&](int t, hipStream_t q) {
        if (use_absm && ((am.kit_mask >> hk.tpl[t].kit_slot) & 1u)) {
            AbsMidArgs at = am;
            at.bests = c->mid_bests + (size_t)t * slots; at.tpl = t; at.den = hk.tpl[t].den; at.kit_slot = hk.tpl[t].kit_slot;
            at.cursor = am.cursor + t;
            const QOptVal wg = qopt_get(QO_MIDDLE_ABS_WGS);
            const QOptVal ow = qopt_get(QO_MIDDLE_ABS_ONE_WAVE);
            const int sk = hk.tpl[t].static_kernel;
            const bool big_enough = slots >= (size_t)abs_cu_count() * 2048 * 11 / 4;
            const bool one = (ow ? atoi(ow) != 0 : big_enough) && qcat_absmid_launch(sk, 1, 0, nullptr, nullptr) != 0;
            const int per_cu = wg ? atoi(wg) : std::max(1, (one ? 8 : 4) / std::max(1, absm_side));
            const unsigned grid = (unsigned)std::min<uint32_t>(am.n_tiles, (uint32_t)(abs_cu_count() * per_cu));
            (void)qcat_absmid_launch(sk, one ? 1 : 2, grid, q, &at);
        }
        MiddleAdapterArgs ma{kp, b->bases, b->offsets, c->mid_sorted, c->mid_len, c->mid_tables,
                             c->mid_bests + (size_t)t * slots, t, use_absm ? c->absm_need : nullptr};
        launch_adapter_middle(hk.tpl[t].static_kernel, dim3(tiles), q, ma);
    });
    {
        const uint32_t fblocks = (uint32_t)std::min<uint64_t>((slots + 255) / 256, 2048);
        hipLaunchKernelGGL(k_adapter_finish, dim3(fblocks), dim3(256), 0, st, kp.kit, c->mid_len, (uint32_t)slots,
                           c->mid_bests, hk.nt, c->mid_recs, sc->jt, (const int32_t*)c->mid_fallback, -1, (const uint8_t*)sc->wspec, sc->jobinfo, (int2*)nullptr, (uint32_t*)nullptr);
    }
    const int nsets = hk.mode == QCAT_MODE_DUAL ? 2 : 1;
    rc = packed_barcode(st, kp, hk, (uint32_t)slots, c->mid_recs, sc, [&](uint32_t max_tiles, const BsPlan* taken, hipStream_t gq) {
        const uint64_t gthreads = (uint64_t)max_tiles * 64 * (WIN_STRIDE / 16);
        hipLaunchKernelGGL(k_mid_gather, dim3((uint32_t)((gthreads + 255) / 256)), dim3(256), 0, gq,
                           b->bases, b->offsets, hk.max_align, c->mid_sorted, c->mid_recs, sc->sorted, sc->jt, nsets,
                           sc->tilebuf, sc->tmeta, taken);
    }, (int16_t*)nullptr, 0u, [](const char*) {});
    if (!rc) rc = jit_take_error();
    if (rc) return set_err(rc, packed_last_error());
    hipLaunchKernelGGL(k_mid_finalize, dim3((n + 255) / 256), dim3(256), 0, st, kp.kit, c->mid_recs, c->mid_slot, n, c->results, c->mid_generic);
    HIPCHK(hipGetLastError());
    return 0;
}

static int max_set_barcodes(const DevKit& hk) {
    int maxb = 1;
    for (int t = 0; t < hk.nt; ++t) for (int s = 0; s < 2; ++s) maxb = std::max(maxb, (int)hk.tpl[t].sets[s].n);
    return maxb;
}

static int tiny_buffers(qcat_ctx* c, size_t n_ends, int maxb) {
    HIPCHK(c->tiny_sc.ensure(std::max<size_t>(n_ends * 2 * (size_t)maxb, (size_t)TINY_MAX_WAVES * 2)));
    HIPCHK(c->tiny_tpl.ensure(std::max<size_t>(n_ends, 4096) * MAX_T * 2));
    return 0;
}

template <int W>
static void launch_simple_packed(hipStream_t st, KitPtrs kp, const uint8_t* win, const int32_t* wlen, uint32_t n_ends, uint32_t n_tiles,
                                 int nch, uint2* part, uint32_t* full) {
    hipLaunchKernelGGL(k_simple_packed<W>, dim3(n_tiles * (uint32_t)nch), dim3(64), 0, st, kp, win, wlen, n_ends, n_tiles, nch, part, full);
}

static int simple_packed_scan(qcat_ctx* c, KitPtrs kp, const DevKit& hk, size_t n_ends, int16_t* dbg_rows, uint32_t row_stride) {
    const DevSet& bs = hk.tpl[0].sets[0];
    const uint32_t n_tiles = (uint32_t)((n_ends + PK_TILE - 1) / PK_TILE);
    const uint32_t target = 8192;
    int nch = (int)std::min<uint32_t>((target + n_tiles - 1) / n_tiles, (uint32_t)bs.n);
    if (dbg_rows) nch = std::min(nch, 8);
    const int per = (bs.n + nch - 1) / nch;
    nch = (bs.n + per - 1) / per;
    int rc;
    if (dbg_rows) { if ((rc = grow(c->simple_full, (size_t)n_tiles * bs.n * 128))) return rc; }
    else {
        if ((rc = grow(c->simple_part, (size_t)n_tiles * nch * 128))) return rc;
        if ((rc = grow(c->simple_redo, n_ends + 1))) return rc;
        HIPCHK(hipMemsetAsync(c->simple_redo, 0, sizeof(uint32_t), c->stream));
    }
    uint32_t* full = dbg_rows ? c->simple_full : nullptr;
    switch (bs.width) {
        case 24: launch_simple_packed<24>(c->stream, kp, c->win, c->wlen, (uint32_t)n_ends, n_tiles, nch, c->simple_part, full); break;
        case 32: launch_simple_packed<32>(c->stream, kp, c->win, c->wlen, (uint32_t)n_ends, n_tiles, nch, c->simple_part, full); break;
        case 40: launch_simple_packed<40>(c->stream, kp, c->win, c->wlen, (uint32_t)n_ends, n_tiles, nch, c->simple_part, full); break;
        case 48: launch_simple_packed<48>(c->stream, kp, c->win, c->wlen, (uint32_t)n_ends, n_tiles, nch, c->simple_part, full); break;
        case 56: launch_simple_packed<56>(c->stream, kp, c->win, c->wlen, (uint32_t)n_ends, n_tiles, nch, c->simple_part, full); break;
        case 64: launch_simple_packed<64>(c->stream, kp, c->win, c->wlen, (uint32_t)n_ends, n_tiles, nch, c->simple_part, full); break;
        default: return set_err(QCAT_ERR_UNSUPPORTED, "simple kit without a width class on the packed path");
    }
    const uint32_t sblocks = (uint32_t)((n_ends + 255) / 256);
    if (dbg_rows) {
        hipLaunchKernelGGL(k_simple_select_rows, dim3(sblocks), dim3(256), 0, c->stream, kp.kit, c->wlen, (uint32_t)n_ends, c->simple_full,
                           c->recs, dbg_rows, row_stride);
    } else {
        hipLaunchKernelGGL(k_simple_select, dim3(sblocks), dim3(256), 0, c->stream, c->wlen, (uint32_t)n_ends, nch, c->simple_part, c->recs, c->simple_redo);
        const uint32_t rblocks = (uint32_t)std::min<size_t>((n_ends + GEN_THREADS - 1) / GEN_THREADS, 1024);
        hipLaunchKernelGGL(k_simple_redo, dim3(rblocks), dim3(GEN_THREADS), 0, c->stream, kp, c->win, c->wlen, c->recs, c->simple_redo);
    }
    return 0;
}

static int scan_resident_impl(qcat_ctx* c, qcat_kit* kit, const qcat_batch* b, bool debug, uint32_t row_stride,
                              bool adapter_only = false, int resume_kit_mask = -1, bool keep_counts = false) {
    if (!c || !kit || !b) return set_err(QCAT_ERR_ARG, "null argument");
    if (b->device != c->device) return set_err(QCAT_ERR_ARG, "batch lives on another device than the context");
    HIPCHK(hipSetDevice(c->device));
    KitOnDevice* kd = nullptr;
    int rc = kit_on_device(kit, c->device, &kd);
    if (rc) return rc;
    const DevKit& hk = kit->hk.dk;
    const int ends = hk.ends == QCAT_ENDS_5P ? 1 : 2;
    const uint32_t n = b->n_reads;
    const size_t n_ends = (size_t)n * ends;
    if (n_ends >= (1ull << 31)) return set_err(QCAT_ERR_UNSUPPORTED, "batch too large (>= 2^31 read ends)");

    if ((rc = grow(c->win, n_ends * WIN_STRIDE + 512))) return rc;
    if ((rc = grow(c->wlen, n_ends))) return rc;
    if ((rc = grow(c->wspec, n_ends))) return rc;
    if ((rc = grow(c->win2, n_ends * WIN2_WORDS + 64 + WIN2_FRONT))) return rc;
    if ((rc = grow(c->recs, n_ends))) return rc;
    if ((rc = grow(c->results, (size_t)n))) return rc;
    if ((rc = grow(c->counts, (size_t)hk.n_buckets))) return rc;
    if (debug) {
        if ((rc = grow(c->dbg_tpl, n_ends * 2 * MAX_T))) return rc;
        if (row_stride && (rc = grow(c->dbg_rows, n_ends * 2 * row_stride))) return rc;
        HIPCHK(hipMemsetAsync(c->dbg_tpl, 0, n_ends * 2 * MAX_T * 4, c->stream));
        if (row_stride) HIPCHK(hipMemsetD16Async((hipDeviceptr_t)c->dbg_rows, (unsigned short)0x8000, n_ends * 2 * row_stride, c->stream));
    }
    c->last_n_reads = n;
    c->last_buckets = hk.n_buckets;
    c->last_kit = adapter_only ? nullptr : kit;
    timing_slot(c);
    const bool packed_kit = hk.fast_ok && !c->force_generic && packed_supported(hk);
    bool use_packed = packed_kit;
    const QOptVal tiny_env = qopt_get(QO_TINY_MAX_ENDS);
    const int tiny_maxb = max_set_barcodes(hk);
    const uint64_t tiny_waves = n_ends * (uint64_t)(hk.nt + tiny_maxb * (hk.mode == QCAT_MODE_DUAL ? 2 : 1));
    const bool tiny_fits = tiny_env ? n_ends <= (uint64_t)std::max<long long>(0, atoll(tiny_env)) : tiny_waves <= (uint64_t)TINY_MAX_WAVES;
    const bool tiny = n_ends > 0 && n_ends <= 4096 && tiny_fits && !opt_on(QO_NO_TINY) && hk.mode != QCAT_MODE_SIMPLE && resume_kit_mask < 0 &&
                      !adapter_only && !c->force_generic && hk.gap_open == hk.gap_extend;
    c->last_tiny_ends = tiny ? (uint32_t)n_ends : 0;
    c->last_fused_ends = 0;
    if (tiny) {
        if ((rc = tiny_buffers(c, (size_t)n_ends, tiny_maxb))) return rc;
        use_packed = false;
    }
    FillScope fills(n != 0 && !opt_on(QO_NO_FILL_MERGE));
    if (!keep_counts) HIPCHK(packed_fill(c->counts, 0, (size_t)hk.n_buckets * 8, c->stream));
    if (n == 0) { HIPCHK(packed_fill_flush(c->stream)); return 0; }
    if (c->timing) HIPCHK(hipEventRecord(c->ev[0], c->stream));
    c->absm_codes_early = false;
    if (hk.scan_middle && !adapter_only && packed_kit && middle_packed_ok(hk) && (rc = absmid_codes_early(c, hk, b, n))) return rc;

    KitPtrs kp{kd->kit, kd->codes, kd->ids, kd->tables};
    g_jit = kd;
    c->packed.prepared = false; c->packed.abs_zeroed = 0; c->packed.redo_zeroed = false;
    if (resume_kit_mask < 0) {
        HIPCHK(packed_fill(c->wspec, 0, n_ends, c->stream));
        c->packed.abs_ready = 0;
        if (g_fill_defer && use_packed && hk.mode != QCAT_MODE_SIMPLE) {
            c->packed.slim = use_packed && !debug && !opt_on(QO_NO_SLIM);
            if ((rc = packed_prepare(c->stream, hk, (uint32_t)n_ends, &c->packed))) return set_err(rc, packed_last_error());
            c->packed.prepared = true;
            if (packed_abs_wanted(hk, (uint32_t)n_ends, true) &&
                (rc = packed_abs_buffers(c->stream, hk, (uint32_t)n_ends, &c->packed))) return set_err(rc, packed_last_error());
        }
        HIPCHK(packed_fill_flush(c->stream));
        c->win2_valid = true;
        bool lazy = use_packed && hk.mode != QCAT_MODE_SIMPLE && hk.adapter_f16 && !opt_on(QO_NO_STATIC) &&
                    !opt_on(QO_NO_STATIC_ADAPTER) && !opt_on(QO_EAGER_BYTES);
        for (int t = 0; t < hk.nt && lazy; ++t) lazy = hk.tpl[t].static_kernel >= 0;
        c->packed.lazy = lazy;
        if (use_packed && hk.mode != QCAT_MODE_SIMPLE && !adapter_only && opt_val(QO_PACK_PLANES, 1) != 0 && packed_abs_wanted(hk, (uint32_t)n_ends, true)) {
            if (c->packed.abs_zeroed != (uint32_t)n_ends && (rc = packed_abs_buffers(c->stream, hk, (uint32_t)n_ends, &c->packed))) return set_err(rc, packed_last_error());
            const uint32_t tiles = ((uint32_t)n_ends + ABS_TILE - 1) / ABS_TILE;
            uint32_t* cursor = reinterpret_cast<uint32_t*>(c->packed.abs_flags.get());
            uint32_t* tile_any = cursor + MAX_T;
            (void)qcat_abs_launch_pack_planes(c->stream, b->bases, b->offsets, n, ends, hk.max_align, c->win, c->wlen, c->wspec, c->win2 + WIN2_FRONT, lazy ? 1 : 0,
                                              c->packed.abs_planes, c->packed.abs_valid, reinterpret_cast<uint8_t*>(tile_any + tiles), tile_any);
            c->packed.abs_ready = (uint32_t)n_ends;
            c->last_fused_ends = (uint32_t)n_ends;
        } else {
            const uint32_t pack_blocks = (uint32_t)((n_ends + PACK_WINDOWS - 1) / PACK_WINDOWS);
            if (ends == 2) hipLaunchKernelGGL(k_pack_windows<2>, dim3(pack_blocks), dim3(PACK_THREADS), 0, c->stream,
                                              b->bases, b->offsets, n, hk.max_align, c->win, c->wlen, c->wspec, c->win2 + WIN2_FRONT, lazy ? 1 : 0);
            else hipLaunchKernelGGL(k_pack_windows<1>, dim3(pack_blocks), dim3(PACK_THREADS), 0, c->stream,
                                    b->bases, b->offsets, n, hk.max_align, c->win, c->wlen, c->wspec, c->win2 + WIN2_FRONT, lazy ? 1 : 0);
        }
        if (lazy) hipLaunchKernelGGL(k_expand_special, dim3((uint32_t)((n_ends + 255) / 256)), dim3(256), 0, c->stream,
                                     b->bases, b->offsets, n, ends, hk.max_align, c->wspec, c->win);
        mark(c, "k_pack_windows");
    }
    if (resume_kit_mask >= 0 && g_fill_defer && use_packed && c->packed.slices_single && hk.mode != QCAT_MODE_SIMPLE) {
        c->packed.slim = use_packed && !debug && !opt_on(QO_NO_SLIM);
        if ((rc = packed_prepare(c->stream, hk, (uint32_t)n_ends, &c->packed))) return set_err(rc, packed_last_error());
        c->packed.prepared = true;
    }
    HIPCHK(packed_fill_flush(c->stream));
    if (hk.mode == QCAT_MODE_SIMPLE && adapter_only) return set_err(QCAT_ERR_ARG, "simple mode has no adapter templates to vote with");
    if (resume_kit_mask >= 0 && !(use_packed && c->packed.slices_single))
        return set_err(QCAT_ERR_UNSUPPORTED, "the adapter pass of this kit cannot be resumed per kit (table or general kernels)");
    c->packed.wspec = c->wspec; c->packed.win = c->win; c->packed.win2 = c->win2_valid ? c->win2 + WIN2_FRONT : nullptr;
    const bool slim = use_packed && !debug && hk.mode != QCAT_MODE_SIMPLE && !opt_on(QO_NO_SLIM);
    c->packed.slim = slim;
    if (hk.mode == QCAT_MODE_SIMPLE && kit->hk.simple_packed && !c->force_generic && !opt_on(QO_NO_SIMPLE_PACKED)) {
        if ((rc = simple_packed_scan(c, kp, hk, n_ends, (debug && row_stride) ? c->dbg_rows : nullptr, row_stride))) return rc;
        mark(c, "k_simple_packed");
    } else if (hk.mode == QCAT_MODE_SIMPLE) {
        uint32_t blocks = (uint32_t)((n_ends + GEN_THREADS - 1) / GEN_THREADS);
        hipLaunchKernelGGL(k_scan_simple, dim3(blocks), dim3(GEN_THREADS), 0, c->stream, kp, c->win, c->wlen, (uint32_t)n_ends, c->recs,
                           (debug && row_stride) ? c->dbg_rows : nullptr, row_stride);
        mark(c, "k_scan_simple");
    } else if (use_packed) {
        rc = packed_scan(c->stream, kp, hk, c->win, c->wlen, (uint32_t)n_ends, c->recs, &c->packed,
                         debug ? c->dbg_tpl : nullptr, (debug && row_stride) ? c->dbg_rows : nullptr, row_stride,
                         [&](const char* nm) { mark(c, nm); }, adapter_only, resume_kit_mask);
        if (rc) return set_err(rc, packed_last_error());
    } else if (tiny) {
        TinyArgs ta{kp, c->win, c->wlen, nullptr, nullptr, (uint32_t)n_ends, c->recs, c->tiny_tpl, c->tiny_sc, (uint32_t)tiny_maxb,
                    debug ? c->dbg_tpl : nullptr, (debug && row_stride) ? c->dbg_rows : nullptr, row_stride, 0};
        hipLaunchKernelGGL(k_tiny_adapter, dim3((uint32_t)n_ends * (uint32_t)hk.nt), dim3(64), 0, c->stream, ta);
        hipLaunchKernelGGL(k_tiny_decide, dim3((uint32_t)((n_ends + 63) / 64)), dim3(64), 0, c->stream, ta);
        hipLaunchKernelGGL(k_tiny_barcode, dim3((uint32_t)tiny_maxb, (uint32_t)n_ends * 2), dim3(64), 0, c->stream, ta);
        hipLaunchKernelGGL(k_tiny_select, dim3((uint32_t)n_ends * 2), dim3(64), 0, c->stream, ta);
        mark(c, "k_scan_tiny");
// ... 32 lines not shown
                MidWaveArgs ma{kp, b->bases, b->offsets, n, c->results, c->mid_generic, c->midw_list, count, MIDW_CAP,
                               c->midw_tpl, c->midw_recs, c->midw_sc, (uint32_t)tiny_maxb};
                hipLaunchKernelGGL(k_midw_list, dim3((n + 255) / 256), dim3(256), 0, c->stream, ma);
                hipLaunchKernelGGL(k_midw_adapter, dim3(1024), dim3(64), 0, c->stream, ma);
                hipLaunchKernelGGL(k_midw_decide, dim3(MIDW_CAP * 2 / 64), dim3(64), 0, c->stream, ma);
                hipLaunchKernelGGL(k_midw_barcode, dim3(4096), dim3(64), 0, c->stream, ma);
                hipLaunchKernelGGL(k_midw_finish, dim3(MIDW_CAP / 64), dim3(64), 0, c->stream, ma);
                c->midw_ran = true;
            }
            hipLaunchKernelGGL(k_scan_middle, dim3((n + GEN_THREADS - 1) / GEN_THREADS), dim3(GEN_THREADS), 0, c->stream,
                               kp, b->bases, b->offsets, n, c->results, only);
            hipLaunchKernelGGL(k_count, dim3(blocks), dim3(256), 0, c->stream, kp, c->results, b->offsets, b->true_len, n, c->counts);
            mark(c, "k_scan_middle");
        }
    }
    HIPCHK(hipGetLastError());
    return 0;
}

extern "C" int qcat_scan_resident(qcat_ctx* c, const qcat_kit* kit, const qcat_batch* b) {
    return scan_resident_impl(c, const_cast<qcat_kit*>(kit), b, false, 0);
}

extern "C" int qcat_ctx_synchronize(qcat_ctx* c) {
    if (!c) return set_err(QCAT_ERR_ARG, "null context");
    HIPCHK(hipSetDevice(c->device));
    HIPCHK(hipStreamSynchronize(c->stream));
    return 0;
}

extern "C" int qcat_ctx_fetch_results(qcat_ctx* c, qcat_result* out, uint32_t n_reads) {
    if (!c || !out) return set_err(QCAT_ERR_ARG, "null argument");
    if (n_reads != c->last_n_reads) return set_err(QCAT_ERR_ARG, "n_reads does not match the last scan");
    HIPCHK(hipSetDevice(c->device));
    if (n_reads) HIPCHK(hipMemcpyAsync(out, c->results, (size_t)n_reads * sizeof(qcat_result), hipMemcpyDeviceToHost, c->stream));
    HIPCHK(hipStreamSynchronize(c->stream));
    return 0;
}

extern "C" int qcat_ctx_fetch_counts(qcat_ctx* c, int64_t* counts, int32_t n_buckets) {
    if (!c || !counts) return set_err(QCAT_ERR_ARG, "null argument");
    if (n_buckets != c->last_buckets) return set_err(QCAT_ERR_ARG, "bucket count does not match the last scan");
    HIPCHK(hipSetDevice(c->device));
    HIPCHK(hipMemcpyAsync(counts, c->counts, (size_t)n_buckets * 8, hipMemcpyDeviceToHost, c->stream));
    HIPCHK(hipStreamSynchronize(c->stream));
    return 0;
}

static int fetch_back(qcat_ctx* c, qcat_result* out, uint32_t n_reads, int64_t* counts_add, int32_t n_buckets) {
    const size_t bytes_rec = (size_t)n_reads * sizeof(qcat_result), off_cnt = (bytes_rec + 63) / 64 * 64;
    const size_t need = off_cnt + (counts_add ? (size_t)n_buckets * 8 : 0);
    if (need > (8u << 20)) {
        int rc = qcat_ctx_fetch_results(c, out, n_reads);
        if (!rc && counts_add) {
            std::vector<int64_t> tmp((size_t)n_buckets);
            rc = qcat_ctx_fetch_counts(c, tmp.data(), n_buckets);
            if (!rc) for (size_t i = 0; i < tmp.size(); ++i) counts_add[i] += tmp[i];
        }
        return rc;
    }
    if (n_reads != c->last_n_reads || (counts_add && n_buckets != c->last_buckets)) return set_err(QCAT_ERR_ARG, "sizes do not match the last scan");
    HIPCHK(hipSetDevice(c->device));
    if (need > c->pin_ret.cap()) {
        HIPCHK(hipStreamSynchronize(c->stream));
        HIPCHK(c->pin_ret.ensure(need + need / 4 + 4096));
    }
    if (n_reads) HIPCHK_DRAIN(c->stream, hipMemcpyAsync(c->pin_ret, c->results, bytes_rec, hipMemcpyDeviceToHost, c->stream));
    if (counts_add) HIPCHK_DRAIN(c->stream, hipMemcpyAsync(c->pin_ret + off_cnt, c->counts, (size_t)n_buckets * 8, hipMemcpyDeviceToHost, c->stream));
    HIPCHK(hipStreamSynchronize(c->stream));
    if (n_reads) memcpy(out, c->pin_ret, bytes_rec);
    if (counts_add) {
        const int64_t* tmp = reinterpret_cast<const int64_t*>(c->pin_ret + off_cnt);
        for (int32_t i = 0; i < n_buckets; ++i) counts_add[i] += tmp[i];
    }
    return 0;
}

extern "C" void* qcat_ctx_stream(qcat_ctx* c) { return c ? (void*)c->stream : nullptr; }
extern "C" int64_t qcat_ctx_tiny_ends(const qcat_ctx* c) { return c ? (int64_t)c->last_tiny_ends : -1; }
extern "C" int qcat_ctx_fused_front(const qcat_ctx* c, uint32_t* out) {
    if (!c || !out) return set_err(QCAT_ERR_ARG, "null argument");
    out[0] = c->last_fused_ends;
    out[1] = qcat_abs_launch_pack_planes(nullptr, nullptr, nullptr, 0, 1, 0, nullptr, nullptr, nullptr, nullptr, 0, nullptr, nullptr, nullptr, nullptr);
    return 0;
}
extern "C" int64_t qcat_ctx_middle_wave_reads(qcat_ctx* c) {
    if (!c) return -1;
    if (!c->midw_ran || !c->midw_list) return 0;
    if (hipSetDevice(c->device) != hipSuccess || hipStreamSynchronize(c->stream) != hipSuccess) return -1;
    uint32_t cnt = 0;
    if (hipMemcpy(&cnt, c->midw_list + 2048, sizeof cnt, hipMemcpyDeviceToHost) != hipSuccess) return -1;
    return (int64_t)std::min<uint32_t>(cnt, 2048u);
}
extern "C" int64_t qcat_ctx_graph_replays(const qcat_ctx* c) { return c ? (int64_t)(c->api_graph.replays + c->scan_graph.replays) : -1; }
extern "C" int qcat_ctx_barcode_bitslice_tiles(qcat_ctx* c, uint32_t* out) {
    if (!c || !out) return set_err(QCAT_ERR_ARG, "null argument");
    out[0] = out[1] = out[2] = 0;
    if (!c->packed.bsplan || !c->packed.bs_last) return 0;
    HIPCHK(hipSetDevice(c->device));
    HIPCHK(hipStreamSynchronize(c->stream));
    BsPlan hp;
    HIPCHK(hipMemcpy(&hp, c->packed.bsplan, sizeof hp, hipMemcpyDeviceToHost));
    for (int b = 0; b < JOB_BINS; ++b) {
        const int cls = b % JOB_CLASSES - (JOB_CLASSES - JOB_HOT);
        if (cls >= 0) out[cls] += hp.count[b];
    }
    return 0;
}
extern "C" int qcat_ctx_middle_bitslice_tiles(qcat_ctx* c, uint32_t* out) {
    if (!c || !out) return set_err(QCAT_ERR_ARG, "null argument");
    out[0] = out[1] = out[2] = out[3] = 0;
    if (!c->absm_last_big) return 0;
    HIPCHK(hipSetDevice(c->device));
    HIPCHK(hipStreamSynchronize(c->stream));
    std::vector<int32_t> rows(c->absm_last_big);
    std::vector<uint8_t> need(c->absm_last_128);
    HIPCHK(hipMemcpy(rows.data(), c->absm_tiles, rows.size() * 4, hipMemcpyDeviceToHost));
    HIPCHK(hipMemcpy(need.data(), c->absm_need, need.size(), hipMemcpyDeviceToHost));
    for (int32_t r : rows) if (r > 0) ++out[0];
    out[1] = c->absm_last_big;
    for (uint8_t f : need) if (f) ++out[2];
    out[3] = c->absm_last_128;
    return 0;
}
extern "C" void* qcat_ctx_counts_devptr(qcat_ctx* c) { return c ? c->counts : nullptr; }
extern "C" void* qcat_ctx_results_devptr(qcat_ctx* c) { return c ? c->results : nullptr; }

extern "C" int qcat_ctx_last_timing(qcat_ctx* c, const char** names, float* ms, int cap) {
    if (!c) return set_err(QCAT_ERR_ARG, "null context");
    if (!c->timing) return 0;
    HIPCHK(hipSetDevice(c->device));
    HIPCHK(hipStreamSynchronize(c->stream));
    const int last = c->ring_used - 1;
    if (last < 0) return 0;
    const int n = std::min(cap, c->ring_marks[last]);
    for (int i = 0; i < n; ++i) { names[i] = c->timed_name[last][i]; ms[i] = 0.f; }
    int scans = 0;
    for (int r = 0; r <= last; ++r) {
        if (c->ring_marks[r] != c->ring_marks[last]) continue;
        bool same = true;
        for (int i = 0; i < n; ++i) same = same && c->timed_name[r][i] == c->timed_name[last][i];
        if (!same) continue;
        for (int i = 0; i < n; ++i) { float t = 0.f; HIPCHK(hipEventElapsedTime(&t, c->evr[r][i], c->evr[r][i + 1])); ms[i] += t; }
        ++scans;
    }
    for (int i = 0; i < n; ++i) ms[i] /= (float)scans;
    c->ring_used = 0; c->n_timed = 0; c->ev = nullptr;
    return n;
}

extern "C" void qcat_batch_destroy(qcat_batch* b) {
    if (!b) return;
    int cur = 0; (void)hipGetDevice(&cur);
    (void)hipSetDevice(b->device);
    if (!b->borrowed) { (void)hipFree(b->bases_alloc); (void)hipFree(b->offsets); (void)hipFree(b->true_len); }
    (void)hipSetDevice(cur);
    delete b;
}

static int batch_alloc(qcat_batch* b, const char* err) {
    hipError_t e1 = hipMalloc((void**)&b->bases_alloc, b->n_bases + 2 * BATCH_SLACK);
    if (e1 == hipSuccess) b->bases = b->bases_alloc + BATCH_SLACK;
    hipError_t e2 = hipMalloc((void**)&b->offsets, ((size_t)b->n_reads + 1) * 8);
    if (e1 != hipSuccess || e2 != hipSuccess) return set_err(QCAT_ERR_NOMEM, err);
    return 0;
}
// ... 975 lines not shown
```

### qcat_amd/native.py

```python
import ctypes as C
import os
import sys
import threading

import numpy as np

ABI_VERSION = 6

R1_STRIPED, R1_SCALAR = 0, 1
SG_R1_SCALAR = 0x100
_R1_NAMES = {"striped": R1_STRIPED, "sg_striped_32": R1_STRIPED, "scalar": R1_SCALAR, "sg": R1_SCALAR}
_r1_rule = [_R1_NAMES.get(os.environ.get("QCAT_R1_RULE", "striped").lower(), R1_STRIPED)]


def set_r1_rule(rule):
    old = _r1_rule[0]
    _r1_rule[0] = _R1_NAMES[rule.lower()] if isinstance(rule, str) else (R1_SCALAR if int(rule) else R1_STRIPED)
    return old


def get_r1_rule():
    return _r1_rule[0]
MODE_EPI2ME, MODE_DUAL, MODE_SIMPLE = 0, 1, 2
ENDS_5P, ENDS_BOTH = 1, 3
# ... 208 lines not shown

try:
    if os.environ.get("QCAT_AMD_NO_PYGLUE"):
        raise ImportError("switched off")
    from . import _pyglue
except ImportError:
    _pyglue = None


def read_views(read_sequences):
    if _pyglue is None or type(read_sequences) is not list:
        return None
    return _pyglue.read_views(read_sequences)


def pack_reads(read_sequences):
    n = len(read_sequences)
    offsets = np.zeros(n + 1, dtype=np.uint64)
    if n and all(type(s) is str for s in read_sequences):
        joined = "".join(read_sequences)
        try:
            raw = joined.encode("ascii")
        except UnicodeEncodeError:
            raw = None
        if raw is not None:
            np.cumsum(np.fromiter(map(len, read_sequences), dtype=np.uint64, count=n), out=offsets[1:])
            bases = np.frombuffer(raw, dtype=np.uint8) if raw else np.zeros(1, dtype=np.uint8)
            return np.ascontiguousarray(bases), offsets
    chunks = []
    total = 0
    for i, s in enumerate(read_sequences):
        if s:
            b = s.encode("latin-1", "replace") if isinstance(s, str) else bytes(s)
            chunks.append(b)
            total += len(b)
        offsets[i + 1] = total
    bases = np.frombuffer(b"".join(chunks), dtype=np.uint8) if total else np.zeros(1, dtype=np.uint8)
    return np.ascontiguousarray(bases), offsets


def _ptr(arr, ctype):
    return arr.ctypes.data_as(C.POINTER(ctype))


class HipLibrary(object):

    _instance = None

    def __init__(self, path=LIB_PATH):
        if not os.path.exists(path):
            raise RuntimeError(
                "qcat_amd: native HIP library not found at {} -- run "
                "`python -c 'import __graft_entry__ as g; g.build()'` (there is no CPU fallback)"
                .format(path))
        lib = C.CDLL(path)
        vp, u32, i32 = C.c_void_p, C.c_uint32, C.c_int32
        sig = {
            "qcat_last_error": (C.c_char_p, []),
            "qcat_abi_version": (C.c_int, []),
            "qcat_backend": (C.c_char_p, []),
            "qcat_set_option": (C.c_int, [C.c_char_p, C.c_int64]),
            "qcat_clear_option": (C.c_int, [C.c_char_p]),
            "qcat_get_option": (C.c_int, [C.c_char_p, C.POINTER(C.c_int64)]),
            "qcat_reset_options": (None, []),
            "qcat_option_count": (C.c_int, []),
            "qcat_option_name": (C.c_char_p, [C.c_int]),
            "qcat_option_doc": (C.c_char_p, [C.c_int]),
            "qcat_device_count": (C.c_int, []),
            "qcat_device_numa_node": (C.c_int, [C.c_int]),
            "qcat_kit_create": (C.c_int, [C.POINTER(KitDesc), C.POINTER(vp)]),
            "qcat_kit_destroy": (None, [vp]),
            "qcat_kit_count_buckets": (C.c_int, [vp]),
            "qcat_kit_partition_bins": (C.c_int, [vp]),
            "qcat_kit_describe": (C.c_int, [vp, C.POINTER(KitInfo)]),
            "qcat_kit_attach_code": (C.c_int, [vp, C.c_char_p, C.c_uint64, C.POINTER(i32), C.POINTER(i32),
                                              C.POINTER(i32), C.POINTER(i32)]),
            "qcat_kit_attach_code_quads": (C.c_int, [vp, C.c_char_p, C.c_uint64, C.POINTER(i32), C.POINTER(i32),
                                                    C.POINTER(i32), C.POINTER(i32), C.POINTER(i32), C.POINTER(i32)]),
            "qcat_ctx_stream": (vp, [vp]),
            "qcat_ctx_graph_replays": (C.c_int64, [vp]),
            "qcat_ctx_barcode_bitslice_tiles": (C.c_int, [vp, C.POINTER(C.c_uint32)]),
            "qcat_ctx_tiny_ends": (C.c_int64, [vp]),
            "qcat_ctx_fused_front": (C.c_int, [vp, C.POINTER(C.c_uint32)]),
            "qcat_ctx_middle_wave_reads": (C.c_int64, [vp]),
            "qcat_ctx_middle_bitslice_tiles": (C.c_int, [vp, C.POINTER(C.c_uint32)]),
            "qcat_ctx_create": (C.c_int, [C.c_int, C.POINTER(vp)]),
            "qcat_ctx_destroy": (None, [vp]),
            "qcat_scan_batch": (C.c_int, [vp, vp, vp, vp, u32, vp, vp]),
            "qcat_scan_debug": (C.c_int, [vp, vp, vp, vp, u32, vp, vp, vp, vp, u32]),
            "qcat_detect_kit": (C.c_int, [vp, vp, vp, vp, u32, vp, vp]),
            "qcat_scan_sequences": (C.c_int, [vp, vp, vp, vp, u32, vp]),
            "qcat_scan_batch_auto": (C.c_int, [vp, vp, vp, vp, u32, vp, vp, C.POINTER(i32), vp, vp]),
            "qcat_scan_batch_auto_ptrs": (C.c_int, [vp, vp, C.c_char_p, C.c_char_p, u32, vp, vp, C.POINTER(i32), vp, vp]),
            "qcat_scan_batches_auto_ptrs": (C.c_int, [vp, vp, C.c_char_p, C.c_char_p, u32, u32, vp, vp, vp]),
            "qcat_batch_upload": (C.c_int, [vp, vp, vp, u32, C.POINTER(vp)]),
            "qcat_batch_synthesize": (C.c_int, [vp, vp, C.POINTER(SynthParams), C.POINTER(vp)]),
            "qcat_batch_destroy": (None, [vp]),
            "qcat_batch_info": (C.c_int, [vp, C.POINTER(u32), C.POINTER(C.c_uint64)]),
            "qcat_batch_download": (C.c_int, [vp, vp, vp, vp]),
            "qcat_synth_read": (C.c_int64, [vp, C.POINTER(SynthParams), C.c_uint64, vp, C.c_uint64]),
            "qcat_scan_resident": (C.c_int, [vp, vp, vp]),
            "qcat_ctx_synchronize": (C.c_int, [vp]),
            "qcat_ctx_fetch_results": (C.c_int, [vp, vp, u32]),
            "qcat_ctx_fetch_counts": (C.c_int, [vp, vp, i32]),
            "qcat_ctx_counts_devptr": (vp, [vp]),
            "qcat_ctx_results_devptr": (vp, [vp]),
            "qcat_batch_partition": (C.c_int, [vp, vp, vp, vp, u32, C.POINTER(vp)]),
            "qcat_ctx_fetch_partition": (C.c_int, [vp, vp, i32, vp]),
            "qcat_ctx_partition_bins_devptr": (vp, [vp]),
            "qcat_ctx_partition_source_devptr": (vp, [vp]),
            "qcat_ctx_last_timing": (C.c_int, [vp, C.POINTER(C.c_char_p), C.POINTER(C.c_float), C.c_int]),
            "qcat_ctx_set_timing": (C.c_int, [vp, C.c_int]),
            "qcat_sg_align": (C.c_int, [vp, vp, vp, vp, vp, u32, i32, i32, vp, i32, vp]),
            "qcat_fastq_open": (C.c_int, [C.c_char_p, C.POINTER(vp), C.POINTER(C.c_uint64), C.POINTER(C.c_uint64)]),
            "qcat_fastq_close": (None, [vp]),
            "qcat_fastq_read_info": (C.c_int, [vp, C.c_uint64, C.POINTER(C.c_uint64), C.POINTER(u32), C.POINTER(C.c_uint64), C.POINTER(u32)]),
            "qcat_fastq_demux": (C.c_int, [vp, vp, vp, C.POINTER(DemuxOpts), vp, vp, C.POINTER(DemuxStats)]),
            "qcat_fastq_demux_stream": (C.c_int, [C.c_char_p, vp, vp, C.POINTER(DemuxOpts), C.POINTER(DemuxHist), C.POINTER(DemuxStats)]),
            "qcat_fastq_batch_offsets": (C.c_int, [C.c_char_p, C.c_uint32, C.c_uint64, C.POINTER(C.POINTER(C.c_uint64)), C.POINTER(C.c_uint64),
                                                   C.POINTER(C.c_uint64), C.POINTER(C.c_uint64)]),
            "qcat_free": (None, [vp]),
            "qcat_fastq_stream_count": (C.c_int, [C.c_char_p, C.c_uint64, C.c_uint32, C.c_int32, C.POINTER(C.c_uint64), C.POINTER(C.c_uint64),
                                                  C.POINTER(C.c_uint64), C.POINTER(C.c_uint32)]),
            "qcat_comm_unique_id": (C.c_int, [vp]),
            "qcat_comm_create": (C.c_int, [vp, C.c_int, C.c_int, vp, C.POINTER(vp)]),
            "qcat_comm_destroy": (None, [vp]),
            "qcat_comm_info": (C.c_int, [vp, C.POINTER(C.c_int), C.POINTER(C.c_int), C.POINTER(C.c_int)]),
            "qcat_counts_allreduce": (C.c_int, [vp, vp]),
            "qcat_comm_allreduce_f64": (C.c_int, [vp, vp, C.POINTER(C.c_double), C.c_int, C.c_int]),
            "qcat_comm_barrier": (C.c_int, [vp, vp]),
        }
        for name, (res, args) in sig.items():
            fn = getattr(lib, name)
            fn.restype = res
            fn.argtypes = args
        backend = (lib.qcat_backend() or b"").decode()
        if backend != "hip" or lib.qcat_abi_version() != ABI_VERSION:
            raise RuntimeError("qcat_amd: {} is not the HIP library of ABI {} (backend {!r}, ABI {}); there is no CPU fallback"
                               .format(path, ABI_VERSION, backend, lib.qcat_abi_version()))
        self.lib = lib
        self.path = path
        self.symbols = sorted(sig)

    @classmethod
    def get(cls):
        if cls._instance is None:
            cls._instance = cls()
        return cls._instance

    def check(self, rc):
        if rc != 0:
            msg = self.lib.qcat_last_error()
            if rc == -5:
                raise IOError("qcat_hip: {}".format((msg or b"").decode("utf-8", "replace")))
            raise RuntimeError("qcat_hip error {}: {}".format(rc, (msg or b"").decode("utf-8", "replace")))


def set_option(name, value=1):
    hip = HipLibrary.get()
    if value is None:
        hip.check(hip.lib.qcat_clear_option(name.encode()))
    else:
        hip.check(hip.lib.qcat_set_option(name.encode(), int(value)))


def get_option(name):
# ... 473 lines not shown
```

Baseline: 341.6 million.

## Fuse adapter finish job emission into the bit-sliced two-template adapter kernel

When the fused two-template bit-sliced adapter kernel runs, its consumer wave now merges the two templates' results, computes the barcode region and job bin, and writes job words, finish words, barcode result placeholders and bin histograms straight from LDS. This skips writing per-end AdapterBest records and having k_adapter_finish reread them for the plain 128-end tiles; finish then runs in a flagged mode that only handles the remaining tiles. The cost is extra work and LDS traffic in the adapter kernel's consumer wave, global atomics for the histogram, and more code paths to keep equivalent. Shared region/bin logic is moved into a common header.

Result: no change. 344.6 million, median of 6 (+0.9%).

```diff
diff --git a/include/qcat_hip.h b/include/qcat_hip.h
--- a/include/qcat_hip.h
+++ b/include/qcat_hip.h
@@ -224,6 +224,7 @@
 int qcat_ctx_barcode_bitslice_tiles(qcat_ctx* ctx, uint32_t out[3]);
 int64_t qcat_ctx_tiny_ends(const qcat_ctx* ctx);
 int qcat_ctx_fused_front(const qcat_ctx* ctx, uint32_t out[2]);
+int qcat_ctx_adapter_emit(qcat_ctx* ctx, uint32_t out[2]);
 int64_t qcat_ctx_middle_wave_reads(qcat_ctx* ctx);
 
 int qcat_ctx_middle_bitslice_tiles(qcat_ctx* ctx, uint32_t out[4]);
diff --git a/qcat_amd/csrc/adapter_rule.h b/qcat_amd/csrc/adapter_rule.h
--- /dev/null
+++ b/qcat_amd/csrc/adapter_rule.h
@@ -0,0 +1,79 @@
+#ifndef QCAT_ADAPTER_RULE_H
+#define QCAT_ADAPTER_RULE_H
+
+#include <stdint.h>
+
+#if defined(__HIPCC__) || defined(__HIPCC_RTC__)
+#define QR_FN __host__ __device__ __forceinline__
+#else
+#define QR_FN inline
+#endif
+
+namespace qk {
+
+constexpr int JOB_CLASSES = 7;
+constexpr int JOB_HOT = 3;
+
+QR_FN void dev_region(int tpl_len, int bc_end, int bc_len, int ext, int stop, int L, int* start_out, int* len_out) {
+    int end_ref = stop - (tpl_len - bc_end) + 1;
+    int start_ref = end_ref - bc_len;
+    start_ref -= (ext < start_ref) ? ext : start_ref;
+    end_ref += (ext < L - end_ref) ? ext : (L - end_ref);
+    int a = start_ref, b = end_ref + 1;
+    if (a < 0) { a += L; if (a < 0) a = 0; }
+    if (b < 0) { b += L; if (b < 0) b = 0; }
+    if (a > L) a = L;
+    if (b > L) b = L;
+    *start_out = a;
+    *len_out = b > a ? b - a : 0;
+}
+
+QR_FN int job_class(int L) { return L <= 48 ? 0 : (L <= 64 ? 1 : (L <= 96 ? 2 : 3)); }
+QR_FN int job_class_hot_of(int bs_ok, int max_align, int bs_off, int hot_len, int short_min, int flag, int L, int start) {
+    if ((flag == 0 || flag == 2) && bs_ok && bs_off >= 0) {
+        const bool interior = flag == 2;
+        if (L == max_align && (!interior || start == 0)) return JOB_CLASSES - 1;
+        if (L == hot_len && !interior) return JOB_CLASSES - 2;
+        if (L < hot_len && L >= short_min && !interior) return JOB_CLASSES - 3;
+    }
+    return job_class(L);
+}
+
+struct FinTpl { int32_t kit_slot, is_double, region_min_raw, len, bc_end[2], bc_len[2], hot_len[2], short_min[2], bs_off[2]; };
+struct FinKit { int32_t dual, nsets, bs_ok, max_align, ext; };
+
+QR_FN int adapter_merge2(int raw0, int den0, int raw1, int den1) {
+    const bool ok0 = -den0 < raw0 * 100, ok1 = -den1 < raw1 * 100;
+    const bool second = ok1 & (!ok0 | (raw0 * den1 < raw1 * den0));
+    return second ? 1 : (ok0 ? 0 : -1);
+}
+
+QR_FN void adapter_end_regions(const FinKit& kk, const FinTpl& p, int best_tpl, int best_raw, int best_end, int L,
+                               int& region_path, int (&region_start)[2], int (&region_len)[2]) {
+    region_path = (kk.dual || p.is_double || (best_tpl >= 0 && best_raw >= p.region_min_raw)) ? 1 : 0;
+    for (int s = 0; s < 2; ++s) {
+        int start = 0, len = 0;
+        if (s < kk.nsets) {
+            if (region_path) dev_region(p.len, p.bc_end[s], p.bc_len[s], kk.ext, best_end, L, &start, &len);
+            else len = L < kk.max_align ? L : kk.max_align;
+        }
+        region_start[s] = start; region_len[s] = len;
+    }
+}
+
+QR_FN uint32_t adapter_job_word(const FinKit& kk, const FinTpl& p, int used_tpl, int s, int flag, bool interior, int region_start, int region_len,
+                                int* bin_out) {
+    *bin_out = -1;
+    if (!(region_len > 0 && !(interior && region_len > kk.max_align))) return 0u;
+    const int bin = (used_tpl * 2 + s) * JOB_CLASSES +
+                    job_class_hot_of(kk.bs_ok, kk.max_align, p.bs_off[s], p.hot_len[s], p.short_min[s], flag, region_len, region_start);
+    *bin_out = bin;
+    return (uint32_t)(region_len < 255 ? region_len : 255) | ((uint32_t)bin << 8) | ((uint32_t)region_start << 16);
+}
+
+QR_FN uint32_t adapter_fin_word(int window_len, int used_tpl, int best_end) {
+    return (uint32_t)(window_len & 0xFF) | ((uint32_t)(used_tpl & 0xFF) << 8) | ((uint32_t)(uint16_t)(int16_t)best_end << 16);
+}
+
+}
+#endif
diff --git a/qcat_amd/csrc/kernels_abs.inc b/qcat_amd/csrc/kernels_abs.inc
--- a/qcat_amd/csrc/kernels_abs.inc
+++ b/qcat_amd/csrc/kernels_abs.inc
@@ -203,6 +203,134 @@
     }
 }
 
+constexpr u32 ABS_EMIT_WORDS = 64u * 33u;
+__device__ __forceinline__ u32 abs_emit_slot(u32 lane, u32 i) { return lane * 33u + i; }
+__device__ __forceinline__ void abs_lds_fence() { asm volatile("s_waitcnt lgkmcnt(0)" ::: "memory"); }
+
+
+template <class P>
+__device__ __forceinline__ void abs_emit(const AbsArgs& A, int tile, int lane_in, u32 keep, const qabs::AbsBorder (&bd)[P::NT], const qabs::AbsLastRow (&lr)[P::NT],
+                                         u32* __restrict__ area, u32* __restrict__ tot) {
+    using namespace qabs;
+    static_assert(P::NT == 2 && ABS_NI == 8 && ABS_NF + 1 == 11, "two templates; a template's 19 planes are rows of one 32 x 32 matrix, bits 19 and 20 of a word are free");
+    const int L = A.rows;
+    int lane = lane_in;
+    asm volatile("" : "+v"(lane));
+    __builtin_amdgcn_sched_barrier(0);
+    if (A.emit_need128[(size_t)tile * (ABS_TILE / PK_TILE) + (lane >> 2)]) keep = 0u;
+    tot[lane] += (u32)__popc(keep);
+    const int den0 = A.den[0], den1 = A.den[1];
+    u32 val[2][ABS_NF + 1], endq[2][ABS_NI];
+    abs_decide(bd[0], lr[0], (unsigned)(L - 1), val[0], endq[0], A.r1_scalar != 0);
+    abs_decide(bd[1], lr[1], (unsigned)(L - 1), val[1], endq[1], A.r1_scalar != 0);
+#pragma unroll
+    for (int t = 0; t < 2; ++t) {
+        u32 w[32];
+        __builtin_amdgcn_sched_barrier(0);
+#pragma unroll
+        for (int q = 0; q < 32; ++q) {
+            if (q <= ABS_NF) w[q] = val[t][q];
+            else if (q < ABS_NF + 1 + ABS_NI) w[q] = endq[t][q - ABS_NF - 1];
+            else w[q] = 0u;
+        }
+        bs_transpose32(w);
+        __builtin_amdgcn_sched_barrier(0);
+#pragma unroll
+        for (int i = 0; i < 32; ++i) {
+            if (i % 8 == 0) __builtin_amdgcn_sched_barrier(0);
+            u32* __restrict__ slot = area + abs_emit_slot((u32)lane, (u32)i);
+            if (t == 0) { *slot = w[i]; continue; }
+            const u32 w0 = *slot;
+            const int raw0 = (int)(w0 & 0x7FFu) - (2 * P::M0 + 1), raw1 = (int)(w[i] & 0x7FFu) - (2 * P::M1 + 1);
+            const int win = adapter_merge2(raw0, den0, raw1, den1);
+            *slot = win == 1 ? (w[i] | (1u << 19)) : (win == 0 ? w0 : (1u << 20));
+        }
+    }
+    const DevKit* __restrict__ kit = A.emit_kit;
+    const FinTpl pa = fin_tpl_of(kit->tpl[A.tpl[0]]), pb = fin_tpl_of(kit->tpl[A.tpl[1]]);
+    FinKit kk;
+    kk.dual = 0; kk.nsets = 1;
+    kk.bs_ok = kit->bs_ok; kk.max_align = kit->max_align; kk.ext = kit->ext;
+    unsigned long long cnt0 = 0ull, cnt1 = 0ull;
+#pragma unroll 1
+    for (int i = 0; i < 32; ++i) {
+        if (!((keep >> i) & 1u)) continue;
+        u32* __restrict__ slot = area + abs_emit_slot((u32)lane, (u32)i);
+        const u32 m = *slot;
+        const bool none = (m >> 20) & 1u, second = (m >> 19) & 1u;
+        const bool used1 = none ? A.emit_last != 0 : second;
+        const int best_tpl = none ? -1 : (second ? A.tpl[1] : A.tpl[0]);
+        const int best_raw = none ? -1 : (int)(m & 0x7FFu) - (second ? 2 * P::M1 + 1 : 2 * P::M0 + 1);
+        const int best_end = none ? -1 : (int)((m >> 11) & 0xFFu);
+        FinTpl p;
+        p.kit_slot = 0; p.is_double = used1 ? pb.is_double : pa.is_double; p.region_min_raw = used1 ? pb.region_min_raw : pa.region_min_raw;
+        p.len = used1 ? pb.len : pa.len;
+#pragma unroll
+        for (int s = 0; s < 2; ++s) {
+            p.bc_end[s] = used1 ? pb.bc_end[s] : pa.bc_end[s]; p.bc_len[s] = used1 ? pb.bc_len[s] : pa.bc_len[s];
+            p.hot_len[s] = used1 ? pb.hot_len[s] : pa.hot_len[s]; p.short_min[s] = used1 ? pb.short_min[s] : pa.short_min[s];
+            p.bs_off[s] = used1 ? pb.bs_off[s] : pa.bs_off[s];
+        }
+        const int used_tpl = used1 ? A.tpl[1] : A.tpl[0];
+        int region_path, rs[2], rl[2], bin;
+        adapter_end_regions(kk, p, best_tpl, best_raw, best_end, L, region_path, rs, rl);
+        const u32 ji = adapter_job_word(kk, p, used_tpl, 0, 0, false, rs[0], rl[0], &bin);
+        const unsigned long long inc = (unsigned long long)(ji != 0u) << (8 * (ji ? bin - used_tpl * 2 * JOB_CLASSES : 0));
+        cnt0 += used1 ? 0ull : inc; cnt1 += used1 ? inc : 0ull;
+        *slot = (ji ? ji : (u32)(used_tpl * 2 * JOB_CLASSES) << 8) | ((u32)(best_end + 1) << 24);
+    }
+    abs_lds_fence();
+    const u32 e0 = (u32)tile * (u32)ABS_TILE;
+    const u32 second_bin = (u32)(A.tpl[1] * 2 * JOB_CLASSES);
+#pragma unroll 1
+    for (int k = 0; k < ABS_TILE / 256; ++k) {
+        const u32 j = (u32)k * 256u + (u32)lane * 4u;
+        const u32 e = e0 + j;
+        if (e >= A.n_ends || A.emit_need128[e / PK_TILE]) continue;
+        u32 ji[4], fw[4];
+#pragma unroll
+        for (int q = 0; q < 4; ++q) {
+            const u32 w = area[abs_emit_slot(j >> 5, (j & 31u) + (u32)q)];
+            ji[q] = (w & 0xFFu) ? (w & 0x00FFFFFFu) : 0u;
+            const int used_tpl = ((w >> 8) & 0xFFu) >= second_bin ? A.tpl[1] : A.tpl[0];
+            fw[q] = adapter_fin_word(L, used_tpl, (int)(w >> 24) - 1);
+        }
+        if (e + 4 <= A.n_ends) {
+            *reinterpret_cast<uint4*>(A.emit_jobinfo + e) = make_uint4(ji[0], ji[1], ji[2], ji[3]);
+            *reinterpret_cast<uint4*>(A.emit_fin + e) = make_uint4(fw[0], fw[1], fw[2], fw[3]);
+            uint4* __restrict__ br = reinterpret_cast<uint4*>(A.emit_bcres + e);
+            br[0] = make_uint4(0xFFFFFFFFu, 0u, 0xFFFFFFFFu, 0u);
+            br[1] = make_uint4(0xFFFFFFFFu, 0u, 0xFFFFFFFFu, 0u);
+        } else {
+            for (int q = 0; q < 4 && e + q < A.n_ends; ++q) { A.emit_jobinfo[e + q] = ji[q]; A.emit_fin[e + q] = fw[q]; A.emit_bcres[e + q] = make_int2(-1, 0); }
+        }
+    }
+    abs_lds_fence();
+    area[0 * 64 + lane] = (u32)cnt0; area[1 * 64 + lane] = (u32)(cnt0 >> 32);
+    area[2 * 64 + lane] = (u32)cnt1; area[3 * 64 + lane] = (u32)(cnt1 >> 32);
+    abs_lds_fence();
+    if (lane < 2 * JOB_CLASSES) {
+        const int cls = lane % JOB_CLASSES;
+        const u32* __restrict__ src = area + ((lane / JOB_CLASSES) * 2 + (cls >> 2)) * 64;
+        const int sh = (cls & 3) * 8;
+        u32 sum = 0;
+#pragma unroll 8
+        for (int l = 0; l < 64; ++l) sum += (src[(l + lane) & 63] >> sh) & 0xFFu;
+        tot[64 + lane] += sum;
+    }
+    abs_lds_fence();
+}
+
+__device__ __forceinline__ void abs_emit_flush(const AbsArgs& A, int lane, const u32* __restrict__ tot) {
+    const u32 bin_total = tot[64 + lane];
+    if (lane < 2 * JOB_CLASSES && bin_total)
+        atomicAdd(&A.emit_jt->hist[A.tpl[lane / JOB_CLASSES] * 2 * JOB_CLASSES + lane % JOB_CLASSES], bin_total);
+    u32 n = tot[lane];
+#pragma unroll
+    for (int off = 32; off > 0; off >>= 1) n += (u32)__shfl_xor((int)n, off, 64);
+    if (lane == 0 && n) atomicAdd(&A.emit_jt->emit_ends[0], n);
+}
+
 template <class P>
 __device__ __forceinline__ void abs_body(const AbsArgs& A) {
     using namespace qabs;
@@ -210,8 +338,10 @@
     constexpr int PL = 2 + 4 * NH;
     constexpr int LR_WORDS = 2 * ABS_NF + 1;
     static_assert(NH * LR_WORDS <= ABS_R * PL, "the last-row hand-over must fit a ring buffer");
+    static_assert(NT != 2 || ABS_EMIT_WORDS <= (u32)(ABS_R * PL * 64), "the emit step works in one ring buffer");
     __shared__ u32 ring[2][ABS_R * PL * 64];
     __shared__ int s_item[2][2];
+    __shared__ u32 s_emit_tot[NT == 2 ? 128 : 1];
     const int lane = threadIdx.x & 63, wave = uni((int)(threadIdx.x >> 6));
     const int L = A.rows;
     const int NB = (L + ABS_R - 1) / ABS_R;
@@ -281,6 +411,8 @@
     } else {
         u32 h[P::NC1][4];
         AbsBorder bd[NT];
+        if (NT == 2) { s_emit_tot[lane] = 0u; s_emit_tot[64 + lane] = 0u; }
+        const bool emit = NT == 2 && ABS_NI == 8 && A.emit_jobinfo != nullptr;
         __syncthreads();
         for (int step = 1;; ++step) {
             const int buf = (step - 1) & 1;
@@ -324,13 +456,19 @@
                 }
                 P::last1(h, li, lr);
                 const u32 keep = A.valid[(size_t)tile * 64 + lane];
+                if constexpr (NT == 2 && ABS_NI == 8) {
+                    if (emit) abs_emit<P>(A, tile, lane, keep, bd, lr, ring[buf], s_emit_tot);
+                }
+                int lane_d = lane;
+                asm volatile("" : "+v"(lane_d));
 #pragma unroll
                 for (int t = 0; t < NT; ++t) {
+                    if (emit) break;
                     u32 val[ABS_NF + 1], endq[ABS_NI];
                     abs_decide(bd[t], lr[t], (unsigned)(L - 1), val, endq, A.r1_scalar != 0);
                     const int M = t == 0 ? P::M0 : P::M1;
                     const int den = A.den[t], tpl = A.tpl[t];
-                    AdapterBest* __restrict__ out = A.bests[t] + (size_t)tile * ABS_TILE + (size_t)lane * 32;
+                    AdapterBest* __restrict__ out = A.bests[t] + (size_t)tile * ABS_TILE + (size_t)lane_d * 32;
                     for (int bit = 0; bit < 32; ++bit) {
                         if (!((keep >> bit) & 1u)) continue;
                         int v = 0, e = 0;
@@ -340,7 +478,7 @@
                         for (int q = 0; q < ABS_NI; ++q) e |= (int)((endq[q] >> bit) & 1u) << q;
                         const int score = v - 2 * M - 1;
                         if (A.dbg_tpl) {
-                            const size_t eidx = (size_t)tile * ABS_TILE + (size_t)lane * 32 + (size_t)bit;
+                            const size_t eidx = (size_t)tile * ABS_TILE + (size_t)lane_d * 32 + (size_t)bit;
                             A.dbg_tpl[(eidx * 2 + 0) * MAX_T + tpl] = score;
                             A.dbg_tpl[(eidx * 2 + 1) * MAX_T + tpl] = e;
                         }
@@ -351,6 +489,9 @@
                 }
             }
             __syncthreads();
+        }
+        if constexpr (NT == 2 && ABS_NI == 8) {
+            if (emit) abs_emit_flush(A, lane, s_emit_tot);
         }
     }
 }
diff --git a/qcat_amd/csrc/kernels_generic.inc b/qcat_amd/csrc/kernels_generic.inc
--- a/qcat_amd/csrc/kernels_generic.inc
+++ b/qcat_amd/csrc/kernels_generic.inc
@@ -127,20 +127,9 @@
     out[a] = r;
 }
 
-__device__ __host__ inline void dev_region(int tpl_len, int bc_end, int bc_len, int ext, int stop, int L,
-                                           int* start_out, int* len_out) {
-    int end_ref = stop - (tpl_len - bc_end) + 1;
-    int start_ref = end_ref - bc_len;
-    start_ref -= (ext < start_ref) ? ext : start_ref;
-    end_ref += (ext < L - end_ref) ? ext : (L - end_ref);
-    int a = start_ref, b = end_ref + 1;
-    if (a < 0) { a += L; if (a < 0) a = 0; }
-    if (b < 0) { b += L; if (b < 0) b = 0; }
-    if (a > L) a = L;
-    if (b > L) b = L;
-    *start_out = a;
-    *len_out = b > a ? b - a : 0;
-}
+}
+#include "adapter_rule.h"
+namespace qk {
 
 __global__ void __launch_bounds__(GEN_THREADS)
 k_scan_generic(KitPtrs kp, const uint8_t* __restrict__ win, const int32_t* __restrict__ wlen,
diff --git a/qcat_amd/csrc/kernels_packed.inc b/qcat_amd/csrc/kernels_packed.inc
--- a/qcat_amd/csrc/kernels_packed.inc
+++ b/qcat_amd/csrc/kernels_packed.inc
@@ -42,22 +42,10 @@
 constexpr int PK_WAVES = 1;
 constexpr int PK_TILE = 128;
 constexpr int PK_ROWS = 152;
-constexpr int JOB_CLASSES = 7;
-constexpr int JOB_HOT = 3;
 constexpr int JOB_GROUPS = MAX_T * 2;
 constexpr int JOB_BINS = JOB_GROUPS * JOB_CLASSES;
 static_assert(JOB_BINS <= 256, "a bin index is one byte of a job word (k_adapter_finish)");
 
-__device__ __host__ __forceinline__ int job_class(int L) { return L <= 48 ? 0 : (L <= 64 ? 1 : (L <= 96 ? 2 : 3)); }
-__device__ __forceinline__ int job_class_hot_of(int bs_ok, int max_align, int bs_off, int hot_len, int short_min, int flag, int L, int start) {
-    if ((flag == 0 || flag == 2) && bs_ok && bs_off >= 0) {
-        const bool interior = flag == 2;
-        if (L == max_align && (!interior || start == 0)) return JOB_CLASSES - 1;
-        if (L == hot_len && !interior) return JOB_CLASSES - 2;
-        if (L < hot_len && L >= short_min && !interior) return JOB_CLASSES - 3;
-    }
-    return job_class(L);
-}
 __device__ __forceinline__ u32 make_sel(u32 qb) {
     return (((qb << 12) | qb) & 0x000F000Fu) | 0x0C000C00u;
 }
@@ -70,6 +58,7 @@
     uint32_t cursor[JOB_BINS];
     uint32_t group_tile_start[JOB_GROUPS + 1];
     uint32_t unit_cursor[JOB_GROUPS][8][32];
+    uint32_t emit_ends[2];
 };
 
 enum { TBL_VGPR = 1, TBL_LDS = 2 };
@@ -221,34 +210,40 @@
     for (int hf = 0; hf < 2; ++hf) if (valid[hf]) bests[e2[hf]] = best[hf];
 }
 
+__host__ __device__ __forceinline__ FinTpl fin_tpl_of(const DevTpl& p) {
+    FinTpl f;
+    f.kit_slot = p.kit_slot; f.is_double = p.is_double; f.region_min_raw = p.region_min_raw; f.len = p.len;
+#pragma unroll
+    for (int s = 0; s < 2; ++s) {
+        f.bc_end[s] = p.bc_end[s]; f.bc_len[s] = p.bc_len[s];
+        f.hot_len[s] = p.sets[s].hot_len; f.short_min[s] = p.sets[s].bs_short_min; f.bs_off[s] = p.sets[s].bs_off;
+    }
+    return f;
+}
+
+template <bool FLAGGED>
 __global__ void __launch_bounds__(256)
 k_adapter_finish(const DevKit* __restrict__ k, const int32_t* __restrict__ wlen, uint32_t n_ends,
                  const AdapterBest* __restrict__ bests, int n_slices, EndRec* __restrict__ recs,
                  JobTables* __restrict__ jt, const int32_t* __restrict__ fallback_tpl, int kit_mask,
                  const uint8_t* __restrict__ wspec, uint32_t* __restrict__ jobinfo, int2* __restrict__ bcres,
-                 uint32_t* __restrict__ fin, const int32_t* __restrict__ kit_slot_dev = nullptr, uint32_t slot_span = 0) {
+                 uint32_t* __restrict__ fin, const int32_t* __restrict__ kit_slot_dev = nullptr, uint32_t slot_span = 0,
+                 const uint8_t* __restrict__ only128 = nullptr) {
     if (kit_slot_dev && !slot_span) kit_mask = *kit_slot_dev;
     __shared__ uint32_t hist[JOB_BINS];
-    struct FinTpl { int32_t kit_slot, is_double, region_min_raw, len, bc_end[2], bc_len[2], hot_len[2], short_min[2], bs_off[2]; };
+    __shared__ uint32_t s_took;
     __shared__ FinTpl s_tpl[MAX_T];
     if (threadIdx.x < JOB_BINS) hist[threadIdx.x] = 0;
+    if (threadIdx.x == 0) s_took = 0;
     const int nt = k->nt;
-    if ((int)threadIdx.x < nt) {
-        const DevTpl& p = k->tpl[threadIdx.x];
-        FinTpl f;
-        f.kit_slot = p.kit_slot; f.is_double = p.is_double; f.region_min_raw = p.region_min_raw; f.len = p.len;
-#pragma unroll
-        for (int s = 0; s < 2; ++s) {
-            f.bc_end[s] = p.bc_end[s]; f.bc_len[s] = p.bc_len[s];
-            f.hot_len[s] = p.sets[s].hot_len; f.short_min[s] = p.sets[s].bs_short_min; f.bs_off[s] = p.sets[s].bs_off;
-        }
-        s_tpl[threadIdx.x] = f;
-    }
+    if ((int)threadIdx.x < nt) s_tpl[threadIdx.x] = fin_tpl_of(k->tpl[threadIdx.x]);
     __syncthreads();
-    const bool dual = k->mode == QCAT_MODE_DUAL;
-    const int nsets = dual ? 2 : 1;
-    const int bs_ok = k->bs_ok, max_align = k->max_align, ext = k->ext;
-    for (uint32_t e = blockIdx.x * blockDim.x + threadIdx.x; e < n_ends; e += gridDim.x * blockDim.x) {
+    FinKit kk;
+    kk.dual = k->mode == QCAT_MODE_DUAL ? 1 : 0;
+    kk.nsets = kk.dual ? 2 : 1;
+    kk.bs_ok = k->bs_ok; kk.max_align = k->max_align; kk.ext = k->ext;
+    const int nsets = kk.nsets;
+    auto one_end = [&](uint32_t e) {
         AdapterBest cs[MAX_T];
 #pragma unroll
         for (int sl = 0; sl < MAX_T; ++sl) if (sl < n_slices) cs[sl] = bests[(size_t)sl * n_ends + e];
@@ -273,26 +268,35 @@
         if (kit_mask >= 0) while (last > 0 && s_tpl[last].kit_slot != kit_mask) --last;
         r.used_tpl = b.tpl < 0 ? (fallback_tpl ? fb : last) : b.tpl;
         const FinTpl& p = s_tpl[r.used_tpl];
-        r.region_path = (dual || p.is_double || (b.tpl >= 0 && b.raw >= p.region_min_raw)) ? 1 : 0;
-        for (int s = 0; s < 2; ++s) { r.region_start[s] = 0; r.region_len[s] = 0; r.bc_idx[s] = -1; r.bc_raw[s] = 0; }
-        for (int s = 0; s < nsets; ++s) {
-            if (r.region_path) dev_region(p.len, p.bc_end[s], p.bc_len[s], ext, b.end, L, &r.region_start[s], &r.region_len[s]);
-            else { r.region_start[s] = 0; r.region_len[s] = L < max_align ? L : max_align; }
-            uint32_t ji = 0;
-            if (r.region_len[s] > 0 && !(fallback_tpl != nullptr && r.region_len[s] > max_align)) {
-                const int bin = (r.used_tpl * 2 + s) * JOB_CLASSES +
-                                job_class_hot_of(bs_ok, max_align, p.bs_off[s], p.hot_len[s], p.short_min[s], flag, r.region_len[s], r.region_start[s]);
-                atomicAdd(&hist[bin], 1u);
-                ji = (uint32_t)min(r.region_len[s], 255) | ((uint32_t)bin << 8) | ((uint32_t)r.region_start[s] << 16);
-            }
+        adapter_end_regions(kk, p, b.tpl, b.raw, b.end, L, r.region_path, r.region_start, r.region_len);
+        for (int s = 0; s < 2; ++s) { r.bc_idx[s] = -1; r.bc_raw[s] = 0; }
+#pragma unroll
+        for (int s = 0; s < 2; ++s) {
+            if (s >= nsets) break;
+            int bin;
+            const uint32_t ji = adapter_job_word(kk, p, r.used_tpl, s, flag, fallback_tpl != nullptr, r.region_start[s], r.region_len[s], &bin);
+            if (ji) atomicAdd(&hist[bin], 1u);
             jobinfo[(size_t)e * nsets + s] = ji;
             if (bcres) bcres[(size_t)e * nsets + s] = make_int2(-1, 0);
         }
-        if (fin) fin[e] = (uint32_t)(r.window_len & 0xFF) | ((uint32_t)(r.used_tpl & 0xFF) << 8) | ((uint32_t)(uint16_t)(int16_t)r.best_end << 16);
+        if (fin) fin[e] = adapter_fin_word(r.window_len, r.used_tpl, r.best_end);
         else recs[e] = r;
+    };
+    if constexpr (FLAGGED) {
+        const uint32_t n128 = (n_ends + PK_TILE - 1) / PK_TILE;
+        uint32_t took = 0;
+        for (uint32_t t = blockIdx.x * 2u + (threadIdx.x >> 7); t < n128; t += gridDim.x * 2u) {
+            if (!only128[t]) continue;
+            const uint32_t e = t * PK_TILE + (threadIdx.x & 127u);
+            if (e < n_ends) { one_end(e); ++took; }
+        }
+        if (took) atomicAdd(&s_took, took);
+    } else {
+        for (uint32_t e = blockIdx.x * blockDim.x + threadIdx.x; e < n_ends; e += gridDim.x * blockDim.x) one_end(e);
     }
     __syncthreads();
     if (threadIdx.x < JOB_BINS && hist[threadIdx.x]) atomicAdd(&jt->hist[threadIdx.x], hist[threadIdx.x]);
+    if (FLAGGED && threadIdx.x == 0 && s_took) atomicAdd(&jt->emit_ends[1], s_took);
 }
 
 __global__ void k_job_offsets(JobTables* jt) {
@@ -844,6 +848,13 @@
     int32_t* dbg_tpl;
     int32_t prio;
     int32_t r1_scalar;
+    uint32_t* emit_jobinfo;
+    uint32_t* emit_fin;
+    int2* emit_bcres;
+    JobTables* emit_jt;
+    const uint8_t* emit_need128;
+    int32_t emit_last;
+    const DevKit* emit_kit;
 };
 struct StaticAdapterMulti {
     StaticAdapterArgs common;
diff --git a/qcat_amd/csrc/options.h b/qcat_amd/csrc/options.h
--- a/qcat_amd/csrc/options.h
+++ b/qcat_amd/csrc/options.h
@@ -33,6 +33,8 @@
     X(NO_ADAPTER_BITSLICE, "1: the adapter scan on the binary16 kernels") \
     X(ADAPTER_BITSLICE_MIN, "read ends from which the bit-sliced adapter scan is taken") \
     X(ABS_STAGES, "2 / 4: one form of the adapter plans for every batch size") \
+    X(ABS_NO_SPLIT, "1: medium batches keep the fused two-template plan") \
+    X(ADAPTER_EMIT, "0: the fused two-template adapter plan leaves every read end to k_adapter_finish instead of writing the jobs of the plain 128-end tiles itself") \
     X(FORCE_GENERIC, "1 at context creation: the general int32 kernel for everything") \
     X(MIDDLE_GENERIC, "1: --detect-middle on the general kernel") \
     X(MIDDLE_NO_ABS, "1: the interior adapter scan on the binary16 kernel") \
@@ -65,7 +67,6 @@
     X(PACK_PLANES, "0: windows and adapter letter planes of a big batch as two kernels (k_pack_windows, k_abs_planes) instead of one (k_pack_planes)") \
     X(FIN_BLOCKS, "blocks of k_finalize") \
     X(FINISH_BLOCKS, "blocks of k_adapter_finish") \
-    X(ABS_NO_SPLIT, "1: medium batches keep the fused two-template plan") \
     X(ABS_PRIO, "issue priority rotation of the bit-sliced adapter kernels") \
     X(ADAPTER_REVERSE, "1: the side-by-side adapter launches in reverse order") \
     X(MIDDLE_NO_BITSLICE, "1: the interior's barcode jobs on the binary16 kernels") \
diff --git a/qcat_amd/csrc/packed_host.inc b/qcat_amd/csrc/packed_host.inc
--- a/qcat_amd/csrc/packed_host.inc
+++ b/qcat_amd/csrc/packed_host.inc
@@ -48,6 +48,8 @@
     uint32_t abs_zeroed = 0;
     const int32_t* kit_slot_dev = nullptr;
     uint32_t kit_slot_span = 0;
+    bool emit_on = false;
+    uint32_t finish_ends = 0;
     bool prepared = false;
     bool redo_zeroed = false;
     static constexpr int NAUX = 11;
@@ -227,13 +229,21 @@
 }
 
 static inline int packed_adapter_finish(hipStream_t stream, KitPtrs kp, const uint8_t* , const int32_t* wlen,
-                                        uint32_t n_ends, EndRec* recs, PackedScratch* sc, int kit_mask) {
+                                        uint32_t n_ends, EndRec* recs, PackedScratch* sc, int kit_mask,
+                                        const uint8_t* only128 = nullptr ) {
     const QOptVal fb_env = qopt_get(QO_FINISH_BLOCKS);
     const uint32_t fblocks = std::min<uint32_t>((n_ends + 255) / 256, fb_env ? (uint32_t)std::max(1, atoi(fb_env)) : 1024u);
     const int32_t* slot_dev = kit_mask == RESUME_KIT_ON_DEVICE ? sc->kit_slot_dev : nullptr;
-    hipLaunchKernelGGL(k_adapter_finish, dim3(fblocks), dim3(256), 0, stream, kp.kit, wlen, n_ends, sc->bests, sc->n_slices, recs, sc->jt,
-                       (const int32_t*)nullptr, slot_dev ? -1 : kit_mask, sc->wspec, sc->jobinfo, sc->slim ? sc->bcres : nullptr, sc->fin_only ? sc->fin : nullptr,
-                       slot_dev, slot_dev ? sc->kit_slot_span : 0u);
+    if (only128)
+        hipLaunchKernelGGL(k_adapter_finish<true>, dim3(fblocks), dim3(256), 0, stream, kp.kit, wlen, n_ends, sc->bests, sc->n_slices, recs, sc->jt,
+                           (const int32_t*)nullptr, slot_dev ? -1 : kit_mask, sc->wspec, sc->jobinfo, sc->slim ? sc->bcres : nullptr, sc->fin_only ? sc->fin : nullptr,
+                           slot_dev, slot_dev ? sc->kit_slot_span : 0u, only128);
+    else
+        hipLaunchKernelGGL(k_adapter_finish<false>, dim3(fblocks), dim3(256), 0, stream, kp.kit, wlen, n_ends, sc->bests, sc->n_slices, recs, sc->jt,
+                           (const int32_t*)nullptr, slot_dev ? -1 : kit_mask, sc->wspec, sc->jobinfo, sc->slim ? sc->bcres : nullptr, sc->fin_only ? sc->fin : nullptr,
+                           slot_dev, slot_dev ? sc->kit_slot_span : 0u, (const uint8_t*)nullptr);
+    sc->emit_on = only128 != nullptr;
+    sc->finish_ends = n_ends;
     hipError_t e = hipGetLastError();
     if (e != hipSuccess) return packed_fail("packed kernel launch", e);
     return 0;
@@ -255,6 +265,7 @@
     if ((rc = packed_ensure(sc->bests, (size_t)n_ends * n_slices, "adapter bests"))) return rc;
     const uint32_t tiles = (n_ends + PK_TILE - 1) / PK_TILE;
     const uint32_t blocks = (tiles + PK_WAVES - 1) / PK_WAVES;
+    const uint8_t* emit_need128 = nullptr;
     {
         int slice = 0;
 #define QK_LAUNCH(WW, TT) do { bool present = false; for (int t = 0; t < hk.nt; ++t) present |= table_tpl(t, WW); \
@@ -312,6 +323,10 @@
         const bool abs_ms = stages_env ? atoi(stages_env) == 4 : abs_tiles < (uint32_t)abs_cus * 7u / 2u;
         const bool adapter_reverse = opt_on(QO_ADAPTER_REVERSE);
         const bool adapter_serial = opt_on(QO_ABS_SERIAL) && use_abs;
+        const bool abs_emit = use_abs && ns == 1 && spartner[0] >= 0 && abs_plan[0] && hk.nt == 2 && hk.mode != QCAT_MODE_DUAL &&
+                              hk.tpl[stpl[0]].static_kernel < QCAT_JIT_BASE && sc->slim && sc->fin_only && sc->bcres && sc->fin &&
+                              dbg_tpl == nullptr && hk.max_align <= 150 && opt_val(QO_ADAPTER_EMIT, 1) != 0;
+        emit_need128 = abs_emit ? abs_need128 : nullptr;
         auto adapter_unit = [&](int i0, hipStream_t q) {
             const int i = adapter_reverse ? ns - 1 - i0 : i0;
             const int t = stpl[i];
@@ -321,6 +336,11 @@
             if (abs_plan[i]) {
                 AbsArgs aa{sc->abs_planes, sc->abs_valid, abs_tile_any, {sa.bests, sa.bests2}, {t, spartner[i]},
                            {hk.tpl[t].den, spartner[i] >= 0 ? hk.tpl[spartner[i]].den : 0}, n_ends, abs_tiles, hk.max_align, abs_cursor + i, dbg_tpl, abs_prio, hk.r1_scalar};
+                if (abs_emit) {
+                    aa.emit_jobinfo = sc->jobinfo; aa.emit_fin = sc->fin; aa.emit_bcres = sc->bcres; aa.emit_jt = sc->jt; aa.emit_need128 = abs_need128;
+                    aa.emit_last = spartner[i] == hk.nt - 1 ? 1 : 0;
+                    aa.emit_kit = kp.kit;
+                }
                 const unsigned grid = (unsigned)std::min<uint32_t>(abs_tiles, (uint32_t)abs_cus * 4u);
                 if (spartner[i] >= 0) (void)qcat_abs_launch(0, hk.tpl[t].fused_kernel, grid, q, &aa);
                 else {
@@ -357,7 +377,7 @@
     if ((e = hipGetLastError()) != hipSuccess) return fail("packed kernel launch", e);
     rc = jit_take_error();
     if (rc) return rc;
-    return packed_adapter_finish(stream, kp, win, wlen, n_ends, recs, sc, -1);
+    return packed_adapter_finish(stream, kp, win, wlen, n_ends, recs, sc, -1, emit_need128);
 }
 
 template <class Mark, class Gather>
diff --git a/qcat_amd/csrc/qcat_hip.hip b/qcat_amd/csrc/qcat_hip.hip
--- a/qcat_amd/csrc/qcat_hip.hip
+++ b/qcat_amd/csrc/qcat_hip.hip
@@ -747,7 +747,7 @@
     });
     {
         const uint32_t fblocks = (uint32_t)std::min<uint64_t>((slots + 255) / 256, 2048);
-        hipLaunchKernelGGL(k_adapter_finish, dim3(fblocks), dim3(256), 0, st, kp.kit, c->mid_len, (uint32_t)slots,
+        hipLaunchKernelGGL(k_adapter_finish<false>, dim3(fblocks), dim3(256), 0, st, kp.kit, c->mid_len, (uint32_t)slots,
                            c->mid_bests, hk.nt, c->mid_recs, sc->jt, (const int32_t*)c->mid_fallback, -1, (const uint8_t*)sc->wspec, sc->jobinfo, (int2*)nullptr, (uint32_t*)nullptr);
     }
     const int nsets = hk.mode == QCAT_MODE_DUAL ? 2 : 1;
@@ -860,6 +860,7 @@
                       !adapter_only && !c->force_generic && hk.gap_open == hk.gap_extend;
     c->last_tiny_ends = tiny ? (uint32_t)n_ends : 0;
     c->last_fused_ends = 0;
+    c->packed.emit_on = false; c->packed.finish_ends = 0;
     if (tiny) {
         if ((rc = tiny_buffers(c, (size_t)n_ends, tiny_maxb))) return rc;
         use_packed = false;
@@ -1058,6 +1059,15 @@
     if (!c || !out) return set_err(QCAT_ERR_ARG, "null argument");
     out[0] = c->last_fused_ends;
     out[1] = qcat_abs_launch_pack_planes(nullptr, nullptr, nullptr, 0, 1, 0, nullptr, nullptr, nullptr, nullptr, 0, nullptr, nullptr, nullptr, nullptr);
+    return 0;
+}
+extern "C" int qcat_ctx_adapter_emit(qcat_ctx* c, uint32_t* out) {
+    if (!c || !out) return set_err(QCAT_ERR_ARG, "null argument");
+    out[0] = 0; out[1] = c->packed.finish_ends;
+    if (!c->packed.emit_on || !c->packed.jt) return 0;
+    HIPCHK(hipSetDevice(c->device));
+    HIPCHK(hipStreamSynchronize(c->stream));
+    HIPCHK(hipMemcpy(out, reinterpret_cast<const uint8_t*>(c->packed.jt.get()) + offsetof(JobTables, emit_ends), 2 * sizeof(uint32_t), hipMemcpyDeviceToHost));
     return 0;
 }
 extern "C" int64_t qcat_ctx_middle_wave_reads(qcat_ctx* c) {
diff --git a/qcat_amd/native.py b/qcat_amd/native.py
--- a/qcat_amd/native.py
+++ b/qcat_amd/native.py
@@ -314,6 +314,7 @@
             "qcat_ctx_barcode_bitslice_tiles": (C.c_int, [vp, C.POINTER(C.c_uint32)]),
             "qcat_ctx_tiny_ends": (C.c_int64, [vp]),
             "qcat_ctx_fused_front": (C.c_int, [vp, C.POINTER(C.c_uint32)]),
+            "qcat_ctx_adapter_emit": (C.c_int, [vp, C.POINTER(C.c_uint32)]),
             "qcat_ctx_middle_wave_reads": (C.c_int64, [vp]),
             "qcat_ctx_middle_bitslice_tiles": (C.c_int, [vp, C.POINTER(C.c_uint32)]),
             "qcat_ctx_create": (C.c_int, [C.c_int, C.POINTER(vp)]),
```
